# taiyaki-go/motioncheck_ccm_slam

Hardware: AMD Instinct MI355X
Metric: ORB extract+match Mfeatures/s and GBA iter/s (2k KF, 200k pts) @1/2/4/8 GPU (higher is better)
Workload: dtype u8; 1 GPU; configs[1]: 256 synthetic 752x480 frames per GPU, 8-level pyramid, 1000 features, FAST+quadtree+rBRIEF, then 1000x1000 brute-force Hamming on the 255 consecutive pairs; frames_per_gpu=256

## Files before the change

### include/ccm_hot.h

```cpp
#ifndef CCM_HOT_H
#define CCM_HOT_H

#include <stddef.h>
#include <stdint.h>

#ifdef __cplusplus
extern "C" {
#endif

#define CCM_ABI_VERSION 3

enum {
    CCM_OK = 0,
    CCM_E_ARG = -1,
    CCM_E_DEVICE = -2,
    CCM_E_NOMEM = -3,
    CCM_E_CAPACITY = -4,
    CCM_E_NUMERIC = -5,
    CCM_E_COMM = -6,
    CCM_E_STATE = -7
};

typedef struct ccm_ctx ccm_ctx;

int ccm_abi_version(void);
ccm_ctx* ccm_create(int device, int flags);
void ccm_destroy(ccm_ctx*);
const char* ccm_last_error(const ccm_ctx*);
int ccm_sync(ccm_ctx*);
void* ccm_stream(ccm_ctx*);

enum { CCM_PROF_RESIZE = 0, CCM_PROF_FAST_SCORE, CCM_PROF_CELL_NMS, CCM_PROF_OCTREE, CCM_PROF_ORIENT_DESC,
       CCM_PROF_HAMMING_BF,
       CCM_PROF_BA_LINEARIZE, CCM_PROF_BA_DINV_Y, CCM_PROF_BA_SCHUR_BLOCKS, CCM_PROF_BA_BSCHUR, CCM_PROF_BA_BACKSUB,
       CCM_PROF_COUNT };
int ccm_host_register(ccm_ctx*, void* ptr, size_t bytes);
int ccm_host_unregister(ccm_ctx*, void* ptr);

int ccm_profile_enable(ccm_ctx*, int on);
int ccm_profile_read(ccm_ctx*, float ms[CCM_PROF_COUNT], int32_t launches[CCM_PROF_COUNT]);

typedef struct {
    int   nfeatures;
    float scale_factor;
    int   nlevels;
    int   ini_th_fast;
    int   min_th_fast;
} ccm_orb_params;

#define CCM_MAX_LEVELS 16

typedef struct {
    float x, y;
    float size;
    float angle;
    float response;
    int32_t octave;
    int32_t class_id;
} ccm_keypoint;

int ccm_orb_tables(const ccm_orb_params*, float* scale, float* inv_scale, float* sigma2,
                   float* inv_sigma2, int32_t* features_per_level, int32_t* umax);
int ccm_orb_level_sizes(const ccm_orb_params*, int w, int h, int32_t* level_w, int32_t* level_h);

int ccm_orb_extract(ccm_ctx*, const ccm_orb_params*, const uint8_t* img, int w, int h, int stride,
                    size_t image_stride, int n_images, ccm_keypoint* kps, uint8_t* desc,
                    int32_t* counts, int max_per_image);

int ccm_orb_extract_dev(ccm_ctx*, const ccm_orb_params*, const uint8_t* img_dev, int w, int h,
                        int stride, size_t image_stride, int n_images, int max_per_image);
int ccm_orb_fetch(ccm_ctx*, ccm_keypoint* kps, uint8_t* desc, int32_t* counts);
int ccm_orb_result_dev(ccm_ctx*, const uint8_t** desc_dev, const int32_t** counts_dev,
                       int* max_per_image);

int ccm_orb_debug_level(ccm_ctx*, int image, int level, uint8_t* out, int out_stride);
int ccm_orb_debug_candidates(ccm_ctx*, int image, int level, int32_t* xy, int32_t* score, int max);

int ccm_descriptor_distance(const uint8_t* a, const uint8_t* b);

int ccm_hamming_match(ccm_ctx*, const uint8_t* q, int nq, const uint8_t* t, int nt, int n_pairs,
                      const int32_t* nq_n, const int32_t* nt_n,
                      int32_t* best_idx, int32_t* best_dist, int32_t* second_dist);
int ccm_hamming_match_dev(ccm_ctx*, const uint8_t* q_dev, int nq, size_t q_pair_stride,
                          const uint8_t* t_dev, int nt, size_t t_pair_stride, int n_pairs,
                          const int32_t* nq_n_dev, const int32_t* nt_n_dev,
                          int32_t* best_idx_dev, int32_t* best_dist_dev, int32_t* second_dist_dev);

int ccm_ratio_test(int best_dist, int second_dist, float nnratio, int th, int strict);

typedef struct {
    float nnratio;
    int   check_ori;
    int   th;
    int   strict_th;
} ccm_bow_options;
int ccm_match_bow(ccm_ctx*, const ccm_bow_options*,
                  const uint8_t* desc1, const int32_t* node1, const uint8_t* valid1,
                  const float* angle1, int n1,
                  const uint8_t* desc2, const int32_t* node2, const uint8_t* valid2,
                  const float* angle2, int n2, int32_t* match12);

typedef struct {
    int n;
    const float* kp_x; const float* kp_y; const int32_t* kp_octave;
    const uint8_t* desc;
    float min_x, min_y;
    float inv_w, inv_h;
    int grid_cols, grid_rows;
} ccm_frame_grid;
int ccm_window_candidates(ccm_ctx*, const ccm_frame_grid*, int nq, const float* qx, const float* qy, const float* qr,
                          const int32_t* min_level, const int32_t* max_level, const uint8_t* qdesc, int cap,
                          int32_t* cand_idx, int32_t* cand_dist, int32_t* cand_n);
int ccm_search_by_projection(ccm_ctx*, const ccm_frame_grid*, const float* scale_factors, int n_mp, const uint8_t* in_view,
                             const int32_t* level, const float* view_cos, const float* proj_x, const float* proj_y,
                             const uint8_t* mp_desc, const uint8_t* mp_has_obs, uint8_t* occupied, float th, float nnratio,
                             int32_t* match);

int ccm_search_by_projection_frame(ccm_ctx*, const ccm_frame_grid* current, const float* cur_angle, const float* scale_factors,
                                   int n_last, const uint8_t* valid, const float* u, const float* v, const int32_t* last_octave,
                                   const float* last_angle, const uint8_t* mp_desc, const uint8_t* mp_has_obs, uint8_t* occupied,
                                   float th, int check_ori, int orb_dist, int32_t* match);

int ccm_search_for_initialization(ccm_ctx*, int n1, const int32_t* oct1, const uint8_t* desc1, const float* angle1,
                                  const ccm_frame_grid* f2, const float* angle2, float* prev_matched_xy, int window,
                                  float nnratio, int check_ori, int32_t* matches12);

int ccm_fuse_select(ccm_ctx*, const ccm_frame_grid* kf, const float* scale_factors, const float* inv_level_sigma2, int n_mp,
                    const uint8_t* valid, const float* u, const float* v, const int32_t* level, const uint8_t* mp_desc, float th,
                    int chi2_check, int accept_th, int32_t* best_idx, int32_t* best_dist);

int ccm_fuse_select_batch(ccm_ctx*, int n_kf, const ccm_frame_grid* kfs, const float* scale_factors, const float* inv_level_sigma2,
                          const int32_t* mp_first, const uint8_t* valid, const float* u, const float* v, const int32_t* level,
                          const uint8_t* mp_desc, float th, int chi2_check, int accept_th, int32_t* best_idx, int32_t* best_dist);

int ccm_search_by_sim3(ccm_ctx*, const ccm_frame_grid* kf1, const float* scale_factors1, const ccm_frame_grid* kf2, const float* scale_factors2,
                       const uint8_t* valid1, const float* u1, const float* v1, const int32_t* level1, const uint8_t* mp_desc1,
                       const uint8_t* valid2, const float* u2, const float* v2, const int32_t* level2, const uint8_t* mp_desc2,
                       float th, int32_t* match12);

int ccm_search_by_projection_sim3(ccm_ctx*, const ccm_frame_grid* kf, const float* scale_factors, int n_mp, const uint8_t* valid,
                                  const float* u, const float* v, const int32_t* level, const uint8_t* mp_desc, const uint8_t* observed,
                                  uint8_t* matched, float th, int32_t* best_idx);
int ccm_search_by_projection_sim3_batch(ccm_ctx*, int n_kf, const ccm_frame_grid* kfs, const float* scale_factors, const int32_t* mp_first,
                                        const uint8_t* valid, const float* u, const float* v, const int32_t* level, const uint8_t* mp_desc,
                                        const uint8_t* observed, uint8_t* matched, float th, int32_t* best_idx, int32_t* n_matches);

int ccm_search_for_triangulation(ccm_ctx*, const uint8_t* desc1, const int32_t* node1, const uint8_t* has_mp1, const float* x1, const float* y1,
                                 const float* angle1, int n1, const uint8_t* desc2, const int32_t* node2, const uint8_t* has_mp2,
                                 const float* x2, const float* y2, const float* angle2, const int32_t* octave2, int n2, const float* F12,
                                 float ex, float ey, const float* scale_factors2, const float* level_sigma2_2, int check_ori, int32_t* match12);

typedef struct ccm_vocabulary ccm_vocabulary;
int  ccm_voc_create(ccm_ctx*, int k, int L, int n_nodes, const int32_t* parent, const uint8_t* descriptors, const double* weights,
                    ccm_vocabulary** out);
void ccm_voc_destroy(ccm_vocabulary*);
int  ccm_voc_words(const ccm_vocabulary*);

int ccm_voc_transform(ccm_vocabulary*, const uint8_t* features, int n, int levelsup, int32_t* word_id, double* weight, int32_t* node_id);
int ccm_voc_transform_dev(ccm_vocabulary*, const uint8_t* features_dev, int n, int levelsup, int32_t* word_id, double* weight,
                          int32_t* node_id);

int ccm_bow_vector(int n, const int32_t* word_id, const double* weight, const int32_t* node_id, int weighting, int scoring,
                   int32_t* out_id, double* out_val, int32_t* fv_node);
double ccm_bow_score_l1(int n1, const int32_t* id1, const double* v1, int n2, const int32_t* id2, const double* v2);

int ccm_distinctive_descriptors(ccm_vocabulary*, const uint8_t* desc, const int64_t* first, const int32_t* count, int n_points,
                                int32_t* best);

typedef struct {
    int      n_poses;
    double*  poses;
    const uint8_t* fixed;
    const double*  intr;
    int      n_points;
    double*  points;
    int      n_edges;
    const int32_t* edge_pose;
    const int32_t* edge_point;
    const double*  obs;
    const double*  info;
} ccm_ba_problem;

typedef struct {
    int    iterations;
    double huber_delta;
    int    iterations2;
    double outlier_chi2;
    const volatile uint8_t* stop_flag;
    double pcg_tol;
} ccm_ba_options;

typedef struct {
    int    iterations_done;
    int    trials;
    double chi2_initial;
    double chi2_final;
    double lambda_final;
    int    stopped;
    double t_linearize, t_schur, t_solve, t_update;
    uint8_t* edge_outlier;
    int32_t schur_blocks;
    int64_t schur_pairs;
    int32_t pcg_iterations;
    int32_t pcg_fallbacks;
    int32_t pcg_pipelined;
} ccm_ba_result;

int ccm_ba_solve(ccm_ctx*, ccm_ba_problem*, const ccm_ba_options*, ccm_ba_result*);

typedef struct {
    int            n_frames;
    double*        poses;
    const double*  intr;
    const int32_t* first;
    const double*  points;
    const double*  obs;
    const double*  info;
    uint8_t*       outlier;
    int32_t*       n_inliers;
} ccm_pose_problem;
int ccm_pose_optimize(ccm_ctx*, ccm_pose_problem*);

typedef struct ccm_frame ccm_frame;
int ccm_frame_create(ccm_ctx*, const ccm_frame_grid* g, const float* angle, ccm_frame** out);
int ccm_frame_from_extract(ccm_ctx*, int image, int n, const float* kp_x_un, const float* kp_y_un, float min_x, float min_y,
                           float inv_w, float inv_h, int grid_cols, int grid_rows, ccm_frame** out);
void ccm_frame_destroy(ccm_frame*);
int ccm_frame_size(const ccm_frame*);
int ccm_frame_set_map_points(ccm_frame*, const int32_t* mp_id);
int ccm_frame_get_map_points(ccm_frame*, int32_t* mp_id);
int ccm_frame_debug_grid(ccm_frame*, int32_t* cell_first, int32_t* cell_items);
int ccm_frame_search_by_projection(ccm_ctx*, ccm_frame* f, const float* scale_factors, int n_mp, const uint8_t* in_view,
                                   const int32_t* level, const float* view_cos, const float* proj_x, const float* proj_y,
                                   const uint8_t* mp_desc, const uint8_t* mp_has_obs, const int32_t* query_mp_id,
                                   uint8_t* occupied, float th, float nnratio, int32_t* match);
// ... 99 lines not shown
```

### motioncheck_ccm_slam_amd/_lib.py

```python
from __future__ import annotations

import ctypes as C
import os

import numpy as np

_HERE = os.path.dirname(os.path.abspath(__file__))
LIB_PATH = os.environ.get("CCM_HOT_LIB") or os.path.join(_HERE, "libccm_hot.so")

CCM_OK = 0
ERRORS = {-1: "CCM_E_ARG", -2: "CCM_E_DEVICE", -3: "CCM_E_NOMEM", -4: "CCM_E_CAPACITY",
          -5: "CCM_E_NUMERIC", -6: "CCM_E_COMM", -7: "CCM_E_STATE"}
COMM_ID_BYTES = 128

KP_DTYPE = np.dtype([("x", "f4"), ("y", "f4"), ("size", "f4"), ("angle", "f4"), ("response", "f4"),
                     ("octave", "i4"), ("class_id", "i4")])

SYMBOLS = [
    "ccm_abi_version", "ccm_create", "ccm_destroy", "ccm_last_error", "ccm_sync", "ccm_stream",
    "ccm_host_register", "ccm_host_unregister", "ccm_profile_enable", "ccm_profile_read",
    "ccm_orb_tables", "ccm_orb_level_sizes", "ccm_orb_extract", "ccm_orb_extract_dev", "ccm_orb_fetch",
    "ccm_orb_result_dev", "ccm_orb_debug_level", "ccm_orb_debug_candidates",
    "ccm_descriptor_distance", "ccm_hamming_match", "ccm_hamming_match_dev", "ccm_ratio_test", "ccm_match_bow",
    "ccm_window_candidates", "ccm_search_by_projection", "ccm_search_by_projection_frame", "ccm_search_for_initialization", "ccm_fuse_select", "ccm_fuse_select_batch", "ccm_search_by_sim3", "ccm_search_by_projection_sim3", "ccm_search_by_projection_sim3_batch",
    "ccm_search_for_triangulation", "ccm_voc_create", "ccm_voc_destroy", "ccm_voc_words", "ccm_voc_transform", "ccm_voc_transform_dev",
    "ccm_bow_vector", "ccm_bow_score_l1", "ccm_distinctive_descriptors", "ccm_optimize_sim3", "ccm_optimize_essential_graph", "ccm_correct_map_points",
    "ccm_ba_solve", "ccm_ba_landmark_cuts", "ccm_pose_optimize", "ccm_comm_unique_id", "ccm_comm_init", "ccm_comm_attach", "ccm_comm_destroy",
    "ccm_pose_from_mat4f", "ccm_pose_to_mat4f",
    "ccm_frame_create", "ccm_frame_from_extract", "ccm_frame_destroy", "ccm_frame_size", "ccm_frame_set_map_points",
    "ccm_frame_get_map_points", "ccm_frame_debug_grid", "ccm_frame_search_by_projection", "ccm_frame_search_by_projection_frame",
    "ccm_frame_pose_optimize",
    "ccm_sim3_ransac_iterations", "ccm_sim3_solver_create", "ccm_sim3_solver_destroy", "ccm_sim3_solver_count", "ccm_sim3_solver_iterate",
    "ccm_sim3_solver_find", "ccm_sim3_solver_estimate", "ccm_sim3_solver_state", "ccm_sim3_solver_hypotheses",
]


class CcmError(RuntimeError):
    def __init__(self, code, text=""):
        super().__init__("%s (%d): %s" % (ERRORS.get(code, "CCM_E_?"), code, text))
        self.code = code


class OrbParams(C.Structure):
    _fields_ = [("nfeatures", C.c_int), ("scale_factor", C.c_float), ("nlevels", C.c_int),
                ("ini_th_fast", C.c_int), ("min_th_fast", C.c_int)]


class BowOptions(C.Structure):
    _fields_ = [("nnratio", C.c_float), ("check_ori", C.c_int), ("th", C.c_int), ("strict_th", C.c_int)]


class FrameGrid(C.Structure):
    _fields_ = [("n", C.c_int), ("kp_x", C.c_void_p), ("kp_y", C.c_void_p), ("kp_octave", C.c_void_p), ("desc", C.c_void_p),
                ("min_x", C.c_float), ("min_y", C.c_float), ("inv_w", C.c_float), ("inv_h", C.c_float),
                ("grid_cols", C.c_int), ("grid_rows", C.c_int)]


class BaProblem(C.Structure):
    _fields_ = [("n_poses", C.c_int), ("poses", C.c_void_p), ("fixed", C.c_void_p), ("intr", C.c_void_p),
                ("n_points", C.c_int), ("points", C.c_void_p),
                ("n_edges", C.c_int), ("edge_pose", C.c_void_p), ("edge_point", C.c_void_p),
                ("obs", C.c_void_p), ("info", C.c_void_p)]


class PoseProblem(C.Structure):
    _fields_ = [("n_frames", C.c_int), ("poses", C.c_void_p), ("intr", C.c_void_p), ("first", C.c_void_p),
                ("points", C.c_void_p), ("obs", C.c_void_p), ("info", C.c_void_p), ("outlier", C.c_void_p),
                ("n_inliers", C.c_void_p)]


class Sim3Problem(C.Structure):
    _fields_ = [("n_problems", C.c_int), ("sim3", C.c_void_p), ("fix_scale", C.c_void_p), ("K1", C.c_void_p), ("K2", C.c_void_p),
                ("first", C.c_void_p), ("P1", C.c_void_p), ("P2", C.c_void_p), ("obs1", C.c_void_p), ("obs2", C.c_void_p),
                ("info1", C.c_void_p), ("info2", C.c_void_p), ("th2", C.c_void_p), ("inlier", C.c_void_p), ("n_inliers", C.c_void_p)]


class Sim3RansacProblem(C.Structure):
    _fields_ = [("n_solvers", C.c_int32), ("first", C.c_void_p), ("n1", C.c_void_p), ("fix_scale", C.c_void_p), ("K1", C.c_void_p),
                ("K2", C.c_void_p), ("X1", C.c_void_p), ("X2", C.c_void_p), ("max_err1", C.c_void_p), ("max_err2", C.c_void_p),
                ("indices1", C.c_void_p), ("probability", C.c_double), ("min_inliers", C.c_int32), ("max_iterations", C.c_int32),
                ("draws", C.c_void_p), ("best_inliers", C.c_void_p)]


class EssentialGraph(C.Structure):
    _fields_ = [("n_vertices", C.c_int), ("sim3", C.c_void_p), ("fixed", C.c_void_p), ("fix_scale", C.c_int), ("n_edges", C.c_int),
                ("edge_i", C.c_void_p), ("edge_j", C.c_void_p), ("measurement", C.c_void_p), ("iterations", C.c_int),
                ("iterations_done", C.c_int), ("chi2_initial", C.c_double), ("chi2_final", C.c_double),
                ("factor_blocks", C.c_int), ("factor_rounds", C.c_int), ("solver_bytes", C.c_int64)]


class BaOptions(C.Structure):
    _fields_ = [("iterations", C.c_int), ("huber_delta", C.c_double), ("iterations2", C.c_int),
                ("outlier_chi2", C.c_double), ("stop_flag", C.c_void_p), ("pcg_tol", C.c_double)]


class BaResult(C.Structure):
    _fields_ = [("iterations_done", C.c_int), ("trials", C.c_int), ("chi2_initial", C.c_double),
                ("chi2_final", C.c_double), ("lambda_final", C.c_double), ("stopped", C.c_int),
                ("t_linearize", C.c_double), ("t_schur", C.c_double), ("t_solve", C.c_double),
                ("t_update", C.c_double), ("edge_outlier", C.c_void_p),
                ("schur_blocks", C.c_int32), ("schur_pairs", C.c_int64), ("pcg_iterations", C.c_int32),
                ("pcg_fallbacks", C.c_int32), ("pcg_pipelined", C.c_int32)]


ABI_VERSION = 3
_lib = None


def load():
    global _lib
    if _lib is not None:
        return _lib
    if not os.path.exists(LIB_PATH):
        raise ImportError("%s not found: build it with `make -C motioncheck_ccm_slam_amd/csrc` "
                          "(or __graft_entry__.build()); there is no CPU fallback" % LIB_PATH)
    lib = C.CDLL(LIB_PATH)
    if lib.ccm_abi_version() != ABI_VERSION:
        raise ImportError("%s has ABI version %d, this package mirrors version %d of include/ccm_hot.h: rebuild it"
                          % (LIB_PATH, lib.ccm_abi_version(), ABI_VERSION))
    lib.ccm_create.restype = C.c_void_p
    lib.ccm_create.argtypes = [C.c_int, C.c_int]
    lib.ccm_destroy.argtypes = [C.c_void_p]
    lib.ccm_destroy.restype = None
    lib.ccm_last_error.restype = C.c_char_p
    lib.ccm_last_error.argtypes = [C.c_void_p]
    lib.ccm_sync.argtypes = [C.c_void_p]
    lib.ccm_stream.restype = C.c_void_p
    lib.ccm_stream.argtypes = [C.c_void_p]
    vp = C.c_void_p
    lib.ccm_host_register.argtypes = [vp, vp, C.c_size_t]
    lib.ccm_host_unregister.argtypes = [vp, vp]
    lib.ccm_profile_enable.argtypes = [vp, C.c_int]
    lib.ccm_profile_read.argtypes = [vp, vp, vp]
    lib.ccm_orb_tables.argtypes = [C.POINTER(OrbParams)] + [vp] * 6
    lib.ccm_orb_level_sizes.argtypes = [C.POINTER(OrbParams), C.c_int, C.c_int, vp, vp]
    lib.ccm_orb_extract.argtypes = [vp, C.POINTER(OrbParams), vp, C.c_int, C.c_int, C.c_int, C.c_size_t, C.c_int,
                                    vp, vp, vp, C.c_int]
    lib.ccm_orb_extract_dev.argtypes = [vp, C.POINTER(OrbParams), vp, C.c_int, C.c_int, C.c_int, C.c_size_t,
                                        C.c_int, C.c_int]
    lib.ccm_orb_fetch.argtypes = [vp, vp, vp, vp]
    lib.ccm_orb_result_dev.argtypes = [vp, C.POINTER(vp), C.POINTER(vp), C.POINTER(C.c_int)]
    lib.ccm_orb_debug_level.argtypes = [vp, C.c_int, C.c_int, vp, C.c_int]
    lib.ccm_orb_debug_candidates.argtypes = [vp, C.c_int, C.c_int, vp, vp, C.c_int]
    lib.ccm_descriptor_distance.argtypes = [vp, vp]
    lib.ccm_hamming_match.argtypes = [vp, vp, C.c_int, vp, C.c_int, C.c_int, vp, vp, vp, vp, vp]
    lib.ccm_hamming_match_dev.argtypes = [vp, vp, C.c_int, C.c_size_t, vp, C.c_int, C.c_size_t, C.c_int,
                                          vp, vp, vp, vp, vp]
    lib.ccm_ratio_test.argtypes = [C.c_int, C.c_int, C.c_float, C.c_int, C.c_int]
    lib.ccm_match_bow.argtypes = [vp, C.POINTER(BowOptions), vp, vp, vp, vp, C.c_int, vp, vp, vp, vp, C.c_int, vp]
    lib.ccm_window_candidates.argtypes = [vp, C.POINTER(FrameGrid), C.c_int, vp, vp, vp, vp, vp, vp, C.c_int, vp, vp, vp]
    lib.ccm_search_by_projection.argtypes = [vp, C.POINTER(FrameGrid), vp, C.c_int, vp, vp, vp, vp, vp, vp, vp, vp, C.c_float, C.c_float, vp]
    lib.ccm_search_by_projection_frame.argtypes = [vp, C.POINTER(FrameGrid), vp, vp, C.c_int, vp, vp, vp, vp, vp, vp, vp, vp, C.c_float, C.c_int, C.c_int, vp]
    lib.ccm_search_for_initialization.argtypes = [vp, C.c_int, vp, vp, vp, C.POINTER(FrameGrid), vp, vp, C.c_int, C.c_float, C.c_int, vp]
    lib.ccm_fuse_select.argtypes = [vp, C.POINTER(FrameGrid), vp, vp, C.c_int, vp, vp, vp, vp, vp, C.c_float, C.c_int, C.c_int, vp, vp]
    lib.ccm_fuse_select_batch.argtypes = [vp, C.c_int, vp, vp, vp, vp, vp, vp, vp, vp, vp, C.c_float, C.c_int, C.c_int, vp, vp]
    lib.ccm_search_by_sim3.argtypes = [vp, C.POINTER(FrameGrid), vp, C.POINTER(FrameGrid), vp] + [vp] * 10 + [C.c_float, vp]
    lib.ccm_search_by_projection_sim3.argtypes = [vp, C.POINTER(FrameGrid), vp, C.c_int] + [vp] * 7 + [C.c_float, vp]
    lib.ccm_search_by_projection_sim3_batch.argtypes = [vp, C.c_int, vp, vp, vp] + [vp] * 7 + [C.c_float, vp, vp]
    lib.ccm_search_for_triangulation.argtypes = [vp] * 7 + [C.c_int] + [vp] * 7 + [C.c_int, vp, C.c_float, C.c_float, vp, vp, C.c_int, vp]
    lib.ccm_voc_create.argtypes = [vp, C.c_int, C.c_int, C.c_int, vp, vp, vp, C.POINTER(vp)]
    lib.ccm_voc_destroy.argtypes = [vp]; lib.ccm_voc_destroy.restype = None
    lib.ccm_voc_words.argtypes = [vp]
    lib.ccm_voc_transform.argtypes = [vp, vp, C.c_int, C.c_int, vp, vp, vp]
    lib.ccm_voc_transform_dev.argtypes = [vp, vp, C.c_int, C.c_int, vp, vp, vp]
    lib.ccm_bow_vector.argtypes = [C.c_int, vp, vp, vp, C.c_int, C.c_int, vp, vp, vp]
    lib.ccm_bow_score_l1.argtypes = [C.c_int, vp, vp, C.c_int, vp, vp]; lib.ccm_bow_score_l1.restype = C.c_double
    lib.ccm_distinctive_descriptors.argtypes = [vp, vp, vp, vp, C.c_int, vp]
    lib.ccm_ba_solve.argtypes = [vp, C.POINTER(BaProblem), C.POINTER(BaOptions), C.POINTER(BaResult)]
    lib.ccm_ba_landmark_cuts.argtypes = [vp, C.c_int, C.c_int, C.c_int, vp]
    lib.ccm_comm_attach.argtypes = [vp, vp, C.c_int, C.c_int]
    lib.ccm_pose_optimize.argtypes = [vp, C.POINTER(PoseProblem)]
    lib.ccm_optimize_sim3.argtypes = [vp, C.POINTER(Sim3Problem)]
    lib.ccm_optimize_essential_graph.argtypes = [vp, C.POINTER(EssentialGraph)]
    lib.ccm_correct_map_points.argtypes = [vp, C.c_int, vp, vp, C.c_int, vp, vp]
    lib.ccm_comm_unique_id.argtypes = [vp]
    lib.ccm_comm_init.argtypes = [vp, vp, C.c_int, C.c_int]
    lib.ccm_comm_destroy.argtypes = [vp]
    lib.ccm_pose_from_mat4f.argtypes = [vp, vp]
    lib.ccm_pose_to_mat4f.argtypes = [vp, vp]
    lib.ccm_frame_create.argtypes = [vp, C.POINTER(FrameGrid), vp, C.POINTER(vp)]
    lib.ccm_frame_from_extract.argtypes = [vp, C.c_int, C.c_int, vp, vp, C.c_float, C.c_float, C.c_float, C.c_float, C.c_int, C.c_int,
                                           C.POINTER(vp)]
    lib.ccm_frame_destroy.argtypes = [vp]; lib.ccm_frame_destroy.restype = None
    lib.ccm_frame_size.argtypes = [vp]
    lib.ccm_frame_set_map_points.argtypes = [vp, vp]
    lib.ccm_frame_get_map_points.argtypes = [vp, vp]
    lib.ccm_frame_debug_grid.argtypes = [vp, vp, vp]
    lib.ccm_frame_search_by_projection.argtypes = [vp, vp, vp, C.c_int] + [vp] * 9 + [C.c_float, C.c_float, vp]
    lib.ccm_frame_search_by_projection_frame.argtypes = [vp, vp, vp, vp, C.c_int] + [vp] * 9 + [C.c_float, C.c_int, C.c_int, vp]
    lib.ccm_frame_pose_optimize.argtypes = [vp, vp, C.c_int, vp, vp, C.c_int, vp, vp, vp, vp]
    lib.ccm_sim3_ransac_iterations.argtypes = [C.c_int, C.c_double, C.c_int, C.c_int]
    lib.ccm_sim3_solver_create.argtypes = [vp, C.POINTER(Sim3RansacProblem), C.POINTER(vp)]
    lib.ccm_sim3_solver_destroy.argtypes = [vp]; lib.ccm_sim3_solver_destroy.restype = None
    lib.ccm_sim3_solver_count.argtypes = [vp]
    lib.ccm_sim3_solver_iterate.argtypes = [vp, C.c_int, C.c_int, vp, vp, vp, vp, vp]
    lib.ccm_sim3_solver_find.argtypes = [vp, C.c_int, vp, vp, vp, vp]
    lib.ccm_sim3_solver_estimate.argtypes = [vp, C.c_int, vp, vp, vp]
    lib.ccm_sim3_solver_state.argtypes = [vp, C.c_int, vp, vp, vp, vp]
    lib.ccm_sim3_solver_hypotheses.argtypes = [vp, C.c_int, vp, vp, vp, vp]
    _lib = lib
    return lib


def ptr(a):
    if a is None:
        return None
    if isinstance(a, int):
        return C.c_void_p(a)
    return a.ctypes.data_as(C.c_void_p)


class Context:

    def __init__(self, device: int = 0):
        self.lib = load()
        self.handle = self.lib.ccm_create(int(device), 0)
        if not self.handle:
            raise CcmError(-2, "ccm_create(%d) failed: no such HIP device" % device)
        self.device = device

    def check(self, rc: int) -> int:
        if rc < 0:
            raise CcmError(rc, self.lib.ccm_last_error(self.handle).decode(errors="replace"))
        return rc

    PROF_LABELS = ("k_pyr_resize", "k_fast_score", "k_cell_nms", "k_octree", "k_orient_desc", "k_hamming_bf",
                   "ba_linearize", "ba_dinv_y", "k_sp_schur_blocks", "k_sp_bschur", "k_ba_backsub")

    def host_register(self, arr):
        self.check(self.lib.ccm_host_register(self.handle, ptr(arr), C.c_size_t(arr.nbytes)))

    def host_unregister(self, arr):
        self.check(self.lib.ccm_host_unregister(self.handle, ptr(arr)))

    def profile(self, on: bool):
        self.check(self.lib.ccm_profile_enable(self.handle, int(on)))

    def profile_read(self):
        ms = np.zeros(len(self.PROF_LABELS), "f4"); n = np.zeros(len(self.PROF_LABELS), "i4")
        self.check(self.lib.ccm_profile_read(self.handle, ptr(ms), ptr(n)))
        return {k: (float(ms[i]), int(n[i])) for i, k in enumerate(self.PROF_LABELS)}

    def sync(self):
        self.check(self.lib.ccm_sync(self.handle))

    @property
    def stream(self) -> int:
        return self.lib.ccm_stream(self.handle)

    def close(self):
        if getattr(self, "handle", None):
            self.lib.ccm_destroy(self.handle)
            self.handle = None

    def __del__(self):
        try:
            self.close()
        except Exception:
            pass


_default_ctx = {}


def default_context(device: int = 0) -> Context:
    if device not in _default_ctx:
        _default_ctx[device] = Context(device)
    return _default_ctx[device]
```

### motioncheck_ccm_slam_amd/csrc/match_host.cpp

```cpp
#include "ccm_internal.h"
#include "window_types.h"
#include <algorithm>
#include <climits>
#include <cmath>
#include <numeric>

void match_launch_bf(hipStream_t, const uint8_t* q, long long q_pair_bytes, const uint8_t* t, long long t_pair_bytes,
                     int nq, int nt, int n_pairs, const int* nq_n, const int* nt_n, int n_split, int variant,
                     unsigned* part_best, int* part_second, int* bi, int* bd, int* sd);
void match_launch_ranges(hipStream_t, const uint8_t* d1, const uint8_t* d2, const int* order2, const int* start,
                         const int* len, const long long* off, int n1, unsigned short* dist);
struct BowDev {
    int n_groups, n1;
    const int* ga; const int* gae; const int* gb; const int* gbe;
    const int* ord1; const int* ord2;
    const uint8_t* d1; const uint8_t* d2;
    const uint8_t* valid1; const uint8_t* valid2;
    const float* angle1; const float* angle2;
    uint8_t* taken; int* match12; int* bin_of; int* hist;
    float nnratio; int th, strict_th, check_ori;
};
void match_launch_bow(hipStream_t, const BowDev&);

struct WindowBufs { DevBuf kx, ky, oct, desc, cfirst, citems, qx, qy, qr, minl, maxl, qdesc, ci, cd, cn, sel_i, sel_d, is2, act, qlvl, qflag, flag, out, status, qang, fang, ev,
                           grids, qkf, gkf; };
struct MatchState {
    WindowBufs win;
    DevBuf q, t, nqn, ntn, bi, bd, sd;
    DevBuf part_best, part_second;
    DevBuf d1, d2, order2, start, len, off, dist;
    DevBuf order1, grp[4], bv1, bv2, ba1, ba2, taken, m12, binof, hist;
};
void match_state_free(MatchState* s) { delete s; }

static MatchState* match_state(ccm_ctx* c)
{
    if (!c->match) c->match = new MatchState();
    return c->match;
}
static WindowBufs& window_bufs(ccm_ctx* c) { return match_state(c)->win; }

extern "C" {

int ccm_descriptor_distance(const uint8_t* a, const uint8_t* b)
{
    int d = 0;
    for (int i = 0; i < 8; i++) {
        uint32_t x, y;
        std::memcpy(&x, a + 4 * i, 4);
        std::memcpy(&y, b + 4 * i, 4);
        d += __builtin_popcount(x ^ y);
    }
    return d;
}

int ccm_ratio_test(int best_dist, int second_dist, float nnratio, int th, int strict)
{
    const bool pass = strict ? (best_dist < th) : (best_dist <= th);
    return pass && (static_cast<float>(best_dist) < nnratio * static_cast<float>(second_dist)) ? 1 : 0;
}

int ccm_hamming_match_dev(ccm_ctx* c, const uint8_t* q_dev, int nq, size_t q_pair_stride, const uint8_t* t_dev, int nt,
                          size_t t_pair_stride, int n_pairs, const int32_t* nq_n_dev, const int32_t* nt_n_dev,
                          int32_t* best_idx_dev, int32_t* best_dist_dev, int32_t* second_dist_dev)
{
    RoctxRange roctx_("ccm_hamming_match_dev");
    return ccm_guard(c, "ccm_hamming_match_dev", [&]() -> int {
        if (!c) return CCM_E_ARG;
        if (n_pairs == 0 || nq == 0) return CCM_OK;
        if (n_pairs < 0 || nq < 0 || nt < 0 || nt > 65535 || !q_dev || (!t_dev && nt > 0) || !best_idx_dev || !best_dist_dev || !second_dist_dev)
            return ccm_fail(c, CCM_E_ARG, "bad matcher arguments (nt must be <= 65535)");
        if (((uintptr_t)q_dev | (uintptr_t)t_dev) & 15) return ccm_fail(c, CCM_E_ARG, "descriptor arrays must be 16-byte aligned");
        CCM_HIP(c, hipSetDevice(c->device));
        MatchState& M = *match_state(c);
        static const int env_split = getenv("CCM_BF_SPLIT") ? atoi(getenv("CCM_BF_SPLIT")) : 0;
        static const int variant = getenv("CCM_BF_VARIANT") ? atoi(getenv("CCM_BF_VARIANT")) : 3;
        int n_split = env_split > 0 ? env_split : 1;
        if (env_split <= 0) while (n_split < 8 && (long long)n_pairs * n_split < 1024 && nt / (n_split * 2) >= 128) n_split *= 2;
        if (n_split > 1) {
            CCM_RESERVE(c, M.part_best, (size_t)n_pairs * n_split * nq * 4);
            CCM_RESERVE(c, M.part_second, (size_t)n_pairs * n_split * nq * 4);
        }
        ProfScope ps(c, CCM_PROF_HAMMING_BF);
        match_launch_bf(c->stream, q_dev, (long long)q_pair_stride * 32, t_dev, (long long)t_pair_stride * 32, nq, nt, n_pairs,
                        nq_n_dev, nt_n_dev, n_split, variant, M.part_best.as<unsigned>(), M.part_second.as<int>(),
                        best_idx_dev, best_dist_dev, second_dist_dev);
        CCM_HIP(c, hipGetLastError());
        return CCM_OK;
    });
}

int ccm_hamming_match(ccm_ctx* c, const uint8_t* q, int nq, const uint8_t* t, int nt, int n_pairs, const int32_t* nq_n,
                      const int32_t* nt_n, int32_t* best_idx, int32_t* best_dist, int32_t* second_dist)
{
    RoctxRange roctx_("ccm_hamming_match");
    return ccm_guard(c, "ccm_hamming_match", [&]() -> int {
        if (!c) return CCM_E_ARG;
        if (n_pairs == 0 || nq == 0) return CCM_OK;
        if (n_pairs < 0 || nq < 0 || nt < 0 || !q || (!t && nt > 0) || !best_idx || !best_dist || !second_dist)
            return ccm_fail(c, CCM_E_ARG, "bad matcher arguments");
        CCM_HIP(c, hipSetDevice(c->device));
        MatchState& M = *match_state(c);
        const size_t qb = (size_t)n_pairs * nq * 32, tb = (size_t)n_pairs * nt * 32, ob = (size_t)n_pairs * nq * 4;
        CCM_RESERVE(c, M.q, qb); CCM_RESERVE(c, M.t, std::max<size_t>(tb, 32));
        CCM_RESERVE(c, M.bi, ob); CCM_RESERVE(c, M.bd, ob); CCM_RESERVE(c, M.sd, ob);
        CCM_RESERVE(c, M.nqn, (size_t)n_pairs * 4); CCM_RESERVE(c, M.ntn, (size_t)n_pairs * 4);
        CCM_HIP(c, hipMemcpyAsync(M.q.p, q, qb, hipMemcpyHostToDevice, c->stream));
        if (tb) CCM_HIP(c, hipMemcpyAsync(M.t.p, t, tb, hipMemcpyHostToDevice, c->stream));
        if (nq_n) CCM_HIP(c, hipMemcpyAsync(M.nqn.p, nq_n, (size_t)n_pairs * 4, hipMemcpyHostToDevice, c->stream));
        if (nt_n) CCM_HIP(c, hipMemcpyAsync(M.ntn.p, nt_n, (size_t)n_pairs * 4, hipMemcpyHostToDevice, c->stream));
        int rc = ccm_hamming_match_dev(c, M.q.as<uint8_t>(), nq, nq, M.t.as<uint8_t>(), nt, nt, n_pairs,
                                       nq_n ? M.nqn.as<int32_t>() : nullptr, nt_n ? M.ntn.as<int32_t>() : nullptr,
                                       M.bi.as<int32_t>(), M.bd.as<int32_t>(), M.sd.as<int32_t>());
        if (rc) return rc;
        CCM_HIP(c, hipMemcpyAsync(best_idx, M.bi.p, ob, hipMemcpyDeviceToHost, c->stream));
        CCM_HIP(c, hipMemcpyAsync(best_dist, M.bd.p, ob, hipMemcpyDeviceToHost, c->stream));
        CCM_HIP(c, hipMemcpyAsync(second_dist, M.sd.p, ob, hipMemcpyDeviceToHost, c->stream));
        CCM_HIP(c, hipStreamSynchronize(c->stream));
        return CCM_OK;
    });
}

static void three_maxima(const std::vector<int>* histo, int L, int& ind1, int& ind2, int& ind3)
{
    int max1 = 0, max2 = 0, max3 = 0;
    ind1 = ind2 = ind3 = -1;
    for (int i = 0; i < L; i++) {
        const int s = (int)histo[i].size();
        if (s > max1) { max3 = max2; max2 = max1; max1 = s; ind3 = ind2; ind2 = ind1; ind1 = i; }
        else if (s > max2) { max3 = max2; max2 = s; ind3 = ind2; ind2 = i; }
        else if (s > max3) { max3 = s; ind3 = i; }
    }
    if (max2 < 0.1f * (float)max1) { ind2 = -1; ind3 = -1; }
    else if (max3 < 0.1f * (float)max1) { ind3 = -1; }
}

struct RotHisto {
    static const int HISTO = 30;
    std::vector<int> rot[HISTO];
    void add(float r, int idx)
    {
        if (r < 0.0) r += 360.0f;
        int bin = (int)std::round(r * (1.0f / HISTO));
        if (bin == HISTO) bin = 0;
        rot[bin].push_back(idx);
    }
    std::vector<int> outliers() const
    {
        int i1, i2, i3;
        three_maxima(rot, HISTO, i1, i2, i3);
        std::vector<int> out;
        for (int b = 0; b < HISTO; b++)
            if (b != i1 && b != i2 && b != i3) out.insert(out.end(), rot[b].begin(), rot[b].end());
        return out;
    }
};

struct BowRanges {
    std::vector<int> ord1, ord2, start, len;
    std::vector<long long> off;
    std::vector<unsigned short> dist;
};
static int bow_ranges(ccm_ctx* c, const uint8_t* desc1, const int32_t* node1, const uint8_t* valid1, int n1,
                      const uint8_t* desc2, const int32_t* node2, int n2, BowRanges& R)
{
    MatchState& M = *match_state(c);
    std::vector<int>&ord1 = R.ord1, &ord2 = R.ord2, &start = R.start, &len = R.len;
    std::vector<long long>& off = R.off;
    std::vector<unsigned short>& dist = R.dist;
    ord1.assign(n1, 0); ord2.assign(n2, 0);
    std::iota(ord1.begin(), ord1.end(), 0); std::iota(ord2.begin(), ord2.end(), 0);
    auto by_node = [](const int32_t* node) { return [node](int a, int b) { return node[a] != node[b] ? node[a] < node[b] : a < b; }; };
    std::stable_sort(ord1.begin(), ord1.end(), by_node(node1));
    std::stable_sort(ord2.begin(), ord2.end(), by_node(node2));
    start.assign(n1, 0); len.assign(n1, 0); off.assign(n1 + 1, 0);
    {
        size_t b = 0;
        for (size_t a = 0; a < ord1.size();) {
            const int nd = node1[ord1[a]];
            size_t ae = a; while (ae < ord1.size() && node1[ord1[ae]] == nd) ae++;
            while (b < ord2.size() && node2[ord2[b]] < nd) b++;
            size_t be = b; while (be < ord2.size() && node2[ord2[be]] == nd) be++;
            if (nd >= 0) for (size_t i = a; i < ae; i++) if (valid1[ord1[i]]) { start[ord1[i]] = (int)b; len[ord1[i]] = (int)(be - b); }
            a = ae; b = be;
        }
    }
    for (int i = 0; i < n1; i++) off[i + 1] = off[i] + len[i];
    const long long total = off[n1];
    dist.assign((size_t)std::max<long long>(total, 1), 0);
    if (total > 0) {
        CCM_RESERVE(c, M.d1, (size_t)n1 * 32); CCM_RESERVE(c, M.d2, (size_t)n2 * 32);
        CCM_RESERVE(c, M.order2, (size_t)n2 * 4); CCM_RESERVE(c, M.start, (size_t)n1 * 4); CCM_RESERVE(c, M.len, (size_t)n1 * 4);
        CCM_RESERVE(c, M.off, (size_t)(n1 + 1) * 8); CCM_RESERVE(c, M.dist, (size_t)total * 2);
        CCM_HIP(c, hipMemcpyAsync(M.d1.p, desc1, (size_t)n1 * 32, hipMemcpyHostToDevice, c->stream));
        CCM_HIP(c, hipMemcpyAsync(M.d2.p, desc2, (size_t)n2 * 32, hipMemcpyHostToDevice, c->stream));
        CCM_HIP(c, hipMemcpyAsync(M.order2.p, ord2.data(), (size_t)n2 * 4, hipMemcpyHostToDevice, c->stream));
        CCM_HIP(c, hipMemcpyAsync(M.start.p, start.data(), (size_t)n1 * 4, hipMemcpyHostToDevice, c->stream));
        CCM_HIP(c, hipMemcpyAsync(M.len.p, len.data(), (size_t)n1 * 4, hipMemcpyHostToDevice, c->stream));
        CCM_HIP(c, hipMemcpyAsync(M.off.p, off.data(), (size_t)(n1 + 1) * 8, hipMemcpyHostToDevice, c->stream));
        match_launch_ranges(c->stream, M.d1.as<uint8_t>(), M.d2.as<uint8_t>(), M.order2.as<int>(), M.start.as<int>(),
                            M.len.as<int>(), M.off.as<long long>(), n1, M.dist.as<unsigned short>());
        CCM_HIP(c, hipGetLastError());
        CCM_HIP(c, hipMemcpyAsync(dist.data(), M.dist.p, (size_t)total * 2, hipMemcpyDeviceToHost, c->stream));
        CCM_HIP(c, hipStreamSynchronize(c->stream));
    }
    return CCM_OK;
}

int ccm_match_bow(ccm_ctx* c, const ccm_bow_options* o, const uint8_t* desc1, const int32_t* node1, const uint8_t* valid1,
                  const float* angle1, int n1, const uint8_t* desc2, const int32_t* node2, const uint8_t* valid2,
                  const float* angle2, int n2, int32_t* match12)
{
    RoctxRange roctx_("ccm_match_bow");
    return ccm_guard(c, "ccm_match_bow", [&]() -> int {
        if (!c || !o) return CCM_E_ARG;
        if (n1 < 0 || n2 < 0 || (n1 > 0 && (!desc1 || !node1 || !valid1 || !match12)) || (n2 > 0 && (!desc2 || !node2)) ||
            (o->check_ori && n1 > 0 && n2 > 0 && (!angle1 || !angle2)))
            return ccm_fail(c, CCM_E_ARG, "bad SearchByBoW arguments");
        for (int i = 0; i < n1; i++) match12[i] = -1;
        if (n1 == 0 || n2 == 0) return 0;
        CCM_HIP(c, hipSetDevice(c->device));
        MatchState& M = *match_state(c);
        std::vector<int> ord1(n1), ord2(n2);
        std::iota(ord1.begin(), ord1.end(), 0); std::iota(ord2.begin(), ord2.end(), 0);
        auto by_node = [](const int32_t* node) { return [node](int a, int b) { return node[a] != node[b] ? node[a] < node[b] : a < b; }; };
        std::stable_sort(ord1.begin(), ord1.end(), by_node(node1));
        std::stable_sort(ord2.begin(), ord2.end(), by_node(node2));
        std::vector<int> grp[4];
        {
            size_t pa = 0, pb = 0;
            while (pa < ord1.size() && pb < ord2.size()) {
                const int na = node1[ord1[pa]], nb2 = node2[ord2[pb]];
                if (na < 0) { pa++; continue; }
                if (nb2 < 0) { pb++; continue; }
                if (na < nb2) { while (pa < ord1.size() && node1[ord1[pa]] == na) pa++; continue; }
                if (nb2 < na) { while (pb < ord2.size() && node2[ord2[pb]] == nb2) pb++; continue; }
                size_t ae = pa, be = pb;
                while (ae < ord1.size() && node1[ord1[ae]] == na) ae++;
                while (be < ord2.size() && node2[ord2[be]] == na) be++;
                grp[0].push_back((int)pa); grp[1].push_back((int)ae); grp[2].push_back((int)pb); grp[3].push_back((int)be);
                pa = ae; pb = be;
            }
        }
        const int ng = (int)grp[0].size();
        hipStream_t st = c->stream;
        int rc;
        if ((rc = ccm_upload(c, M.d1, desc1, (size_t)n1 * 32, st)) || (rc = ccm_upload(c, M.d2, desc2, (size_t)n2 * 32, st))) return rc;
        if ((rc = ccm_upload(c, M.order1, ord1.data(), (size_t)n1 * 4, st)) || (rc = ccm_upload(c, M.order2, ord2.data(), (size_t)n2 * 4, st))) return rc;
        for (int k = 0; k < 4; k++) if ((rc = ccm_upload(c, M.grp[k], grp[k].data(), (size_t)ng * 4, st))) return rc;
        if ((rc = ccm_upload(c, M.bv1, valid1, (size_t)n1, st))) return rc;
        if (valid2 && (rc = ccm_upload(c, M.bv2, valid2, (size_t)n2, st))) return rc;
        if (o->check_ori && ((rc = ccm_upload(c, M.ba1, angle1, (size_t)n1 * 4, st)) || (rc = ccm_upload(c, M.ba2, angle2, (size_t)n2 * 4, st)))) return rc;
        CCM_RESERVE(c, M.taken, (size_t)n2); CCM_RESERVE(c, M.m12, (size_t)n1 * 4); CCM_RESERVE(c, M.binof, (size_t)n1 * 4); CCM_RESERVE(c, M.hist, 32 * 4);
        CCM_HIP(c, hipMemsetAsync(M.taken.p, 0, (size_t)n2, st));
        CCM_HIP(c, hipMemsetAsync(M.m12.p, 0xFF, (size_t)n1 * 4, st));
        CCM_HIP(c, hipMemsetAsync(M.hist.p, 0, 32 * 4, st));
        BowDev B{ ng, n1, M.grp[0].as<int>(), M.grp[1].as<int>(), M.grp[2].as<int>(), M.grp[3].as<int>(), M.order1.as<int>(), M.order2.as<int>(),
                  M.d1.as<uint8_t>(), M.d2.as<uint8_t>(), M.bv1.as<uint8_t>(), valid2 ? M.bv2.as<uint8_t>() : nullptr,
                  M.ba1.as<float>(), M.ba2.as<float>(), M.taken.as<uint8_t>(), M.m12.as<int>(), M.binof.as<int>(), M.hist.as<int>(),
                  o->nnratio, o->th, o->strict_th, o->check_ori };
        match_launch_bow(st, B);
        CCM_HIP(c, hipGetLastError());
        int nmatches = 0;
        CCM_HIP(c, hipMemcpyAsync(match12, M.m12.p, (size_t)n1 * 4, hipMemcpyDeviceToHost, st));
        CCM_HIP(c, hipMemcpyAsync(&nmatches, M.hist.as<int>() + 30, 4, hipMemcpyDeviceToHost, st));
        CCM_HIP(c, hipStreamSynchronize(st));
        return nmatches;
    });
}

// ... 659 lines not shown
```

### motioncheck_ccm_slam_amd/csrc/match_kernels.hip

```cpp
#include <hip/hip_runtime.h>
#include <cstdint>

#define BF_TILE 1024

__device__ __forceinline__ int ham256(const uint4& a0, const uint4& a1, const uint4& b0, const uint4& b1)
{
    int d = __popc(a0.x ^ b0.x);
    d += __popc(a0.y ^ b0.y); d += __popc(a0.z ^ b0.z); d += __popc(a0.w ^ b0.w);
    d += __popc(a1.x ^ b1.x); d += __popc(a1.y ^ b1.y); d += __popc(a1.z ^ b1.z); d += __popc(a1.w ^ b1.w);
    return d;
}

template <int THREADS, int QPL>
__global__ __launch_bounds__(THREADS) void k_hamming_bf(
    const uint8_t* __restrict__ q, long long q_pair_bytes, const uint8_t* __restrict__ t, long long t_pair_bytes,
    int nq, int nt, const int* __restrict__ nq_n, const int* __restrict__ nt_n, int n_split,
    unsigned* __restrict__ part_best, int* __restrict__ part_second,
    int* __restrict__ best_idx, int* __restrict__ best_dist, int* __restrict__ second_dist)
{
    __shared__ uint4 tile[BF_TILE * 2];
    const int pair = blockIdx.x / n_split, split = blockIdx.x - pair * n_split, tid = threadIdx.x;
    const int nqp = nq_n ? min(max(nq_n[pair], 0), nq) : nq;
    const int ntp = nt_n ? min(max(nt_n[pair], 0), nt) : nt;
    const int chunk = ((ntp + n_split - 1) / n_split + 63) & ~63;
    const int t_lo = min(split * chunk, ntp), t_hi = min(t_lo + chunk, ntp);
    const uint4* qp = reinterpret_cast<const uint4*>(q + (long long)pair * q_pair_bytes);
    const uint4* tp = reinterpret_cast<const uint4*>(t + (long long)pair * t_pair_bytes);
    const int q_done = ((nqp + QPL * THREADS - 1) / (QPL * THREADS)) * (QPL * THREADS);
    if (n_split == 1 || split == 0)
        for (int qi = q_done + tid; qi < nq; qi += THREADS) {
            if (n_split > 1) {
                for (int sp = 0; sp < n_split; sp++) {
                    const long long o = ((long long)pair * n_split + sp) * nq + qi;
                    part_best[o] = (256u << 16) | 0xFFFFu; part_second[o] = 256;
                }
            } else {
                const long long o = (long long)pair * nq + qi;
                best_idx[o] = -1; best_dist[o] = 256; second_dist[o] = 256;
            }
        }
    for (int qbase = 0; qbase < nqp; qbase += QPL * THREADS) {
        uint4 a0[QPL], a1[QPL];
        unsigned best[QPL]; int sec[QPL];
#pragma unroll
        for (int k = 0; k < QPL; k++) {
            const int qi = qbase + k * THREADS + tid;
            a0[k] = make_uint4(0, 0, 0, 0); a1[k] = a0[k];
            if (qi < nqp) { a0[k] = qp[2 * qi]; a1[k] = qp[2 * qi + 1]; }
            best[k] = (256u << 16) | 0xFFFFu; sec[k] = 256;
        }
        for (int tbase = t_lo; tbase < t_hi; tbase += BF_TILE) {
            const int cnt = min(BF_TILE, t_hi - tbase);
            __syncthreads();
            for (int i = tid; i < 2 * cnt; i += THREADS) tile[i] = tp[2 * tbase + i];
            __syncthreads();
#pragma unroll 2
            for (int j = 0; j < cnt; j++) {
                const uint4 b0 = tile[2 * j], b1 = tile[2 * j + 1];
                const unsigned idx = (unsigned)(tbase + j);
#pragma unroll
                for (int k = 0; k < QPL; k++) {
                    const int d = ham256(a0[k], a1[k], b0, b1);
                    sec[k] = min(sec[k], max(d, (int)(best[k] >> 16)));
                    best[k] = min(best[k], ((unsigned)d << 16) | idx);
                }
            }
        }
#pragma unroll
        for (int k = 0; k < QPL; k++) {
            const int qi = qbase + k * THREADS + tid;
            if (qi >= nq) continue;
            if (n_split > 1) {
                const long long o = ((long long)pair * n_split + split) * nq + qi;
                part_best[o] = best[k]; part_second[o] = sec[k];
            } else {
                const bool live = qi < nqp;
                const long long o = (long long)pair * nq + qi;
                best_idx[o] = (live && (best[k] >> 16) < 256u) ? (int)(best[k] & 0xFFFFu) : -1;
                best_dist[o] = live ? (int)(best[k] >> 16) : 256;
                second_dist[o] = live ? sec[k] : 256;
            }
        }
    }
}

typedef int hm_v4i __attribute__((ext_vector_type(4)));
typedef int hm_v16i __attribute__((ext_vector_type(16)));
#ifndef HM_CB
#define HM_CB 2
#endif
#ifndef HM_WAVES
#define HM_WAVES 4
#endif
#ifndef HM_TT
#define HM_TT 1
#endif
#ifndef HM_WG_PER_CU
#define HM_WG_PER_CU 4
#endif
#define HM_QW (32 * HM_CB)
#define HM_TPB (64 * HM_WAVES)
#define HM_SENT 0x3FFFFFFF
#define HM_MAX_NT 2048

#define HM_BIAS 4352
#define HM_IDX_BITS 11
__device__ __forceinline__ int hm_med3(int a, int b, int c)
{
    return __float_as_int(__builtin_amdgcn_fmed3f(__int_as_float(a), __int_as_float(b), __int_as_float(c)));
}

__device__ __forceinline__ hm_v4i hm_expand16(unsigned hw, int shift)
{
    hm_v4i v;
    const unsigned hs = hw << shift, nm = 15u << shift, bm = 0x01010101u << shift;
    v.x = (int)(__umul24(hs & nm, 0x204081u) & bm); v.y = (int)(__umul24((hs >> 4) & nm, 0x204081u) & bm);
    v.z = (int)(__umul24((hs >> 8) & nm, 0x204081u) & bm); v.w = (int)(__umul24((hs >> 12) & nm, 0x204081u) & bm);
    return v;
}

__global__ __launch_bounds__(HM_TPB, HM_WG_PER_CU * HM_TPB / 256) void k_hamming_mfma(
    const uint8_t* __restrict__ q, long long q_pair_bytes, const uint8_t* __restrict__ t, long long t_pair_bytes,
    int nq, int nt, const int* __restrict__ nq_n, const int* __restrict__ nt_n, int q_blocks,
    int* __restrict__ best_idx, int* __restrict__ best_dist, int* __restrict__ second_dist)
{
    __shared__ hm_v4i frag[2][HM_TT * 8][64];
    __shared__ __attribute__((aligned(16))) int wall[HM_MAX_NT];
    const int pair = blockIdx.x / q_blocks, qblk = blockIdx.x - pair * q_blocks;
    const int tid = threadIdx.x, lane = tid & 63, wv = tid >> 6, h = lane >> 5, r = lane & 31;
    const int nqp = nq_n ? min(max(nq_n[pair], 0), nq) : nq;
    const int ntp = nt_n ? min(max(nt_n[pair], 0), nt) : nt;
    const unsigned* qp = reinterpret_cast<const unsigned*>(q + (long long)pair * q_pair_bytes);
    const unsigned* tp = reinterpret_cast<const unsigned*>(t + (long long)pair * t_pair_bytes);
    const int q0 = qblk * (HM_QW * HM_WAVES) + wv * HM_QW;
    if (qblk * (HM_QW * HM_WAVES) >= nqp) {
        for (int i = tid; i < HM_QW * HM_WAVES; i += HM_TPB) {
            const int qi = qblk * (HM_QW * HM_WAVES) + i;
            if (qi < nq) { const long long o = (long long)pair * nq + qi; best_idx[o] = -1; best_dist[o] = 256; second_dist[o] = 256; }
        }
        return;
    }

    hm_v4i bq[HM_CB][8];
    int pa[HM_CB];
#pragma unroll
    for (int cb = 0; cb < HM_CB; cb++) {
        const int qi = q0 + 32 * cb + r;
        unsigned d[8];
        int pc = 0;
#pragma unroll
        for (int s = 0; s < 8; s++) { d[s] = qi < nqp ? qp[8 * (long long)qi + s] : 0u; pc += __popc(d[s]); }
        pa[cb] = pc;
#pragma unroll
        for (int s = 0; s < 8; s++) bq[cb][s] = hm_expand16((d[s] >> (16 * h)) & 0xFFFFu, 7);
    }
    int m1[HM_CB], m2[HM_CB];
#pragma unroll
    for (int cb = 0; cb < HM_CB; cb++) { m1[cb] = HM_SENT; m2[cb] = HM_SENT; }

    constexpr int HM_FPT = (512 * HM_TT + HM_TPB - 1) / HM_TPB;
    struct Raw { unsigned v[HM_FPT]; };
    auto fetch = [&](int group) {
        Raw x;
#pragma unroll
        for (int j = 0; j < HM_FPT; j++) {
            const int fi = tid + j * HM_TPB, sub = fi >> 9, fw = fi & 511;
            const int tr = (group * HM_TT + sub) * 32 + (fw & 31);
            x.v[j] = (fi < 512 * HM_TT && tr < ntp) ? tp[8 * (long long)tr + ((fw >> 5) & 7)] : 0u;
        }
        return x;
    };
    auto stage = [&](const Raw& x, int buf) {
#pragma unroll
        for (int j = 0; j < HM_FPT; j++) {
            const int fi = tid + j * HM_TPB, sub = fi >> 9, fw = fi & 511;
            if (fi < 512 * HM_TT) frag[buf][8 * sub + ((fw >> 5) & 7)][32 * (fw >> 8) + (fw & 31)] = hm_expand16((x.v[j] >> (16 * (fw >> 8))) & 0xFFFFu, 5);
        }
    };
    for (int tr = tid; tr < ((ntp + 31) & ~31); tr += HM_TPB) {
        int w = HM_SENT;
        if (tr < ntp) {
            const uint4* d = reinterpret_cast<const uint4*>(tp + 8 * (long long)tr);
            const uint4 d0 = d[0], d1 = d[1];
            const int pb = __popc(d0.x) + __popc(d0.y) + __popc(d0.z) + __popc(d0.w) + __popc(d1.x) + __popc(d1.y) + __popc(d1.z) + __popc(d1.w);
            w = ((pb + HM_BIAS) << HM_IDX_BITS) | tr;
        }
        wall[tr] = w;
    }
    const int ntiles = (ntp + 31) >> 5;
    const bool wave_live = q0 < nqp;
    auto mma = [&](int tile, int buf, int sub, hm_v16i (&acc)[HM_CB]) {
        hm_v16i wc;
#pragma unroll
        for (int g = 0; g < 4; g++) {
            const hm_v4i w4 = *reinterpret_cast<const hm_v4i*>(&wall[32 * tile + 8 * g + 4 * h]);
            wc[4 * g] = w4.x; wc[4 * g + 1] = w4.y; wc[4 * g + 2] = w4.z; wc[4 * g + 3] = w4.w;
        }
#pragma unroll
        for (int s = 0; s < 8; s++) {
            const hm_v4i a = frag[buf][8 * sub + s][lane];
#pragma unroll
            for (int cb = 0; cb < HM_CB; cb++) acc[cb] = __builtin_amdgcn_mfma_i32_32x32x32_i8(a, bq[cb][s], s == 0 ? wc : acc[cb], 0, 0, 0);
        }
    };
    auto fold = [&](const hm_v16i (&acc)[HM_CB]) {
#pragma unroll
        for (int i = 0; i < 16; i++)
#pragma unroll
            for (int cb = 0; cb < HM_CB; cb++) {
                const int kx = acc[cb][i];
                m2[cb] = hm_med3(m1[cb], m2[cb], kx); m1[cb] = min(m1[cb], kx);
            }
    };
    const int ngroups = (ntiles + HM_TT - 1) / HM_TT;
    Raw nxt = fetch(0);
    if (ngroups > 0) stage(nxt, 0);
    nxt = fetch(1);
    __syncthreads();
    for (int grp = 0; grp < ngroups; grp++) {
        const int buf = grp & 1;
        if (grp + 1 < ngroups) stage(nxt, buf ^ 1);
        if (grp + 2 < ngroups) nxt = fetch(grp + 2);
        if (wave_live) {
#pragma unroll
            for (int sub = 0; sub < HM_TT; sub++) {
                const int tile = grp * HM_TT + sub;
                if (tile < ntiles) {
                    hm_v16i acc[HM_CB];
                    mma(tile, buf, sub, acc);
                    fold(acc);
                }
            }
        }
        __syncthreads();
    }
#pragma unroll
    for (int cb = 0; cb < HM_CB; cb++) {
        const int o1 = __shfl_xor(m1[cb], 32, 64), o2 = __shfl_xor(m2[cb], 32, 64);
        const int b1 = min(m1[cb], o1);
        const int b2 = min(max(m1[cb], o1), min(m2[cb], o2));
        const int qi = q0 + 32 * cb + r;
        if (h == 0 && qi < nq) {
            const long long o = (long long)pair * nq + qi;
            const bool live = qi < nqp;
            const bool has1 = live && b1 < HM_SENT, has2 = live && b2 < HM_SENT;
            const int bd = has1 ? (b1 >> HM_IDX_BITS) - HM_BIAS + pa[cb] : 256;
            best_idx[o] = bd < 256 ? (b1 & ((1 << HM_IDX_BITS) - 1)) : -1;
            best_dist[o] = bd;
            second_dist[o] = has2 ? (b2 >> HM_IDX_BITS) - HM_BIAS + pa[cb] : 256;
        }
    }
}

__global__ __launch_bounds__(256) void k_hamming_merge(const unsigned* __restrict__ part_best, const int* __restrict__ part_second,
                                                       int n_pairs, int nq, int n_split, const int* __restrict__ nq_n,
                                                       int* __restrict__ best_idx, int* __restrict__ best_dist, int* __restrict__ second_dist)
{
    const long long i = blockIdx.x * 256LL + threadIdx.x;
    if (i >= (long long)n_pairs * nq) return;
    const int pair = (int)(i / nq), qi = (int)(i - (long long)pair * nq);
    const int nqp = nq_n ? min(max(nq_n[pair], 0), nq) : nq;
    unsigned best = (256u << 16) | 0xFFFFu; int sec = 256;
    for (int s = 0; s < n_split; s++) {
        const long long o = ((long long)pair * n_split + s) * nq + qi;
        const unsigned b = part_best[o]; const int sc = part_second[o];
        sec = min(min(sec, sc), max((int)(best >> 16), (int)(b >> 16)));
        best = min(best, b);
    }
    const bool live = qi < nqp;
    best_idx[i] = (live && (best >> 16) < 256u) ? (int)(best & 0xFFFFu) : -1;
    best_dist[i] = live ? (int)(best >> 16) : 256;
    second_dist[i] = live ? sec : 256;
}

__global__ __launch_bounds__(256) void k_hamming_ranges(
    const uint8_t* __restrict__ d1, const uint8_t* __restrict__ d2, const int* __restrict__ order2,
    const int* __restrict__ start, const int* __restrict__ len, const long long* __restrict__ off, int n1,
    unsigned short* __restrict__ dist)
{
    const int i = blockIdx.x * 4 + (threadIdx.x >> 6), lane = threadIdx.x & 63;
    if (i >= n1) return;
    const int L = len[i];
    if (L <= 0) return;
    const uint4* a = reinterpret_cast<const uint4*>(d1) + 2 * (long long)i;
    const uint4 a0 = a[0], a1 = a[1];
    const int s = start[i];
    unsigned short* o = dist + off[i];
    for (int k = lane; k < L; k += 64) {
        const uint4* b = reinterpret_cast<const uint4*>(d2) + 2 * (long long)order2[s + k];
        o[k] = (unsigned short)ham256(a0, a1, b[0], b[1]);
    }
}

struct BowDev {
    int n_groups, n1;
    const int* ga; const int* gae; const int* gb; const int* gbe;
    const int* ord1; const int* ord2;
    const uint8_t* d1b; const uint8_t* d2b;
    const uint8_t* valid1; const uint8_t* valid2;
    const float* angle1; const float* angle2;
    uint8_t* taken; int* match12; int* bin_of; int* hist;
    float nnratio; int th, strict_th, check_ori;
};
__global__ __launch_bounds__(256) void k_bow_greedy(BowDev B)
{
    const int grp = blockIdx.x * 4 + (threadIdx.x >> 6), lane = threadIdx.x & 63;
    if (grp >= B.n_groups) return;
    const int a0 = B.ga[grp], a1 = B.gae[grp], b0 = B.gb[grp], b1 = B.gbe[grp];
    for (int a = a0; a < a1; a++) {
        const int i1 = B.ord1[a];
        if (!B.valid1[i1]) continue;
        const uint4* D1 = reinterpret_cast<const uint4*>(B.d1b); const uint4* D2 = reinterpret_cast<const uint4*>(B.d2b);
        const uint4 q0 = D1[2 * (long long)i1], q1 = D1[2 * (long long)i1 + 1];
        int bd1 = 256, bd2 = 256, bi = -1;
        for (int base = b0; base < b1; base += 64) {
            const int j = base + lane;
            int d = 1 << 20, i2 = -1;
            if (j < b1) {
                i2 = B.ord2[j];
                if (!B.taken[i2] && (!B.valid2 || B.valid2[i2])) d = ham256(q0, q1, D2[2 * (long long)i2], D2[2 * (long long)i2 + 1]);
            }
            unsigned key = ((unsigned)d << 6) | (unsigned)lane;
#pragma unroll
            for (int s = 32; s >= 1; s >>= 1) key = min(key, (unsigned)__shfl_xor((int)key, s, 64));
            const int cb = (int)(key >> 6), cl = (int)(key & 63u);
            int o = lane == cl ? (1 << 20) : d;
#pragma unroll
            for (int s = 32; s >= 1; s >>= 1) o = min(o, __shfl_xor(o, s, 64));
            const int ci2 = __shfl(i2, cl, 64);
            if (cb < bd1) { bd2 = min(bd1, o); bd1 = cb; bi = ci2; }
            else bd2 = min(bd2, cb);
        }
        const bool pass = B.strict_th ? (bd1 < B.th) : (bd1 <= B.th);
        if (bi >= 0 && pass && (float)bd1 < B.nnratio * (float)bd2) {
            if (lane == 0) {
                B.match12[i1] = bi;
                B.taken[bi] = 1;
                if (B.check_ori) {
                    float r = B.angle1[i1] - B.angle2[bi];
                    if (r < 0.0) r += 360.0f;
                    int bin = (int)roundf(r * (1.0f / 30));
                    if (bin == 30) bin = 0;
                    B.bin_of[i1] = bin;
                    atomicAdd(&B.hist[bin], 1);
                }
            }
            __threadfence_block();
        }
    }
}
__global__ __launch_bounds__(256) void k_bow_filter(BowDev B)
{
    __shared__ int keep[3];
    __shared__ int cnt;
    if (threadIdx.x == 0) {
        int max1 = 0, max2 = 0, max3 = 0, ind1 = -1, ind2 = -1, ind3 = -1;
        if (B.check_ori) {
            for (int i = 0; i < 30; i++) {
                const int s = B.hist[i];
                if (s > max1) { max3 = max2; max2 = max1; max1 = s; ind3 = ind2; ind2 = ind1; ind1 = i; }
                else if (s > max2) { max3 = max2; max2 = s; ind3 = ind2; ind2 = i; }
                else if (s > max3) { max3 = s; ind3 = i; }
            }
            if (max2 < 0.1f * (float)max1) { ind2 = -1; ind3 = -1; }
            else if (max3 < 0.1f * (float)max1) ind3 = -1;
        }
        keep[0] = ind1; keep[1] = ind2; keep[2] = ind3; cnt = 0;
    }
    __syncthreads();
    int mine = 0;
    for (int i = threadIdx.x; i < B.n1; i += 256) {
        if (B.match12[i] < 0) continue;
        if (B.check_ori) {
            const int b = B.bin_of[i];
            if (b != keep[0] && b != keep[1] && b != keep[2]) { B.match12[i] = -1; continue; }
        }
        mine++;
    }
    atomicAdd(&cnt, mine);
    __syncthreads();
    if (threadIdx.x == 0) B.hist[30] = cnt;
}
void match_launch_bow(hipStream_t s, const BowDev& B)
{
    if (B.n_groups > 0) hipLaunchKernelGGL(k_bow_greedy, dim3((B.n_groups + 3) / 4), dim3(256), 0, s, B);
    hipLaunchKernelGGL(k_bow_filter, dim3(1), dim3(256), 0, s, B);
}

struct WinGrid {
    int n, cols, rows;
    float min_x, min_y, inv_w, inv_h;
    const float* kx; const float* ky; const int* oct; const uint8_t* desc;
    const int* cell_first; const int* cell_items;
};
template <bool BATCH>
__global__ __launch_bounds__(256) void k_window_candidates(WinGrid G1, const WinGrid* __restrict__ grids, const int* __restrict__ q_kf,
                                                           int nq, const float* __restrict__ qx, const float* __restrict__ qy,
                                                           const float* __restrict__ qr, const int* __restrict__ min_level,
                                                           const int* __restrict__ max_level, const uint8_t* __restrict__ qdesc, int cap,
                                                           int* __restrict__ cand_idx, int* __restrict__ cand_dist, int* __restrict__ cand_n)
{
    const int q = blockIdx.x * 4 + (threadIdx.x >> 6), lane = threadIdx.x & 63;
    if (q >= nq) return;
    const WinGrid G = BATCH ? grids[q_kf[q]] : G1;
// ... 195 lines not shown
                }
            }
            sync(wg);
            const int th = MODE == 0 ? 100 : (MODE == 1 ? 50 : A.orb_dist);
            const int bestDist = k1 == 0xFFFFFFFFu ? 256 : (int)(k1 >> 16);
            int idx1 = -1, idx2 = -1;
            bool safe = false;
            if (unres) {
                if (bestDist > th) safe = true;
                else {
                    const int p1 = (int)(k1 & 0xFFFFu), p2 = (int)(k2 & 0xFFFFu);
                    if (p1 >= WG_REG_CAND) idx1 = ci[p1];
                    if (MODE == 0 && k2 != 0xFFFFFFFFu && p2 >= WG_REG_CAND) idx2 = ci[p2];
#pragma unroll
                    for (int k = 0; k < WG_REG_CAND; k++) {
                        if (k == p1) idx1 = (int)(cand[k] & 0xFFFFu);
                        if (MODE == 0 && k2 != 0xFFFFFFFFu && k == p2) idx2 = (int)(cand[k] & 0xFFFFu);
                    }
                    safe = claim[idx1] == me;
                    if (MODE == 0 && idx2 >= 0) safe = safe && claim[idx2] == me;
                }
            }
            sync(wg);
            if (unres) {
#pragma unroll
                for (int k = 0; k < WG_REG_CAND; k++) if (k < c) claim[cand[k] & 0xFFFFu] = 0x7FFFFFFF;
                for (int k = WG_REG_CAND; k < c; k++) claim[ci[k]] = 0x7FFFFFFF;
            }
            if (unres && safe) {
                unres = false;
                if (bestDist <= th) {
                    if (MODE == 0) {
                        const int bestLevel = octl[idx1], bestLevel2 = idx2 >= 0 ? (int)octl[idx2] : -1;
                        const int bestDist2 = idx2 >= 0 ? (int)(k2 >> 16) : 256;
                        if (!(bestLevel == bestLevel2 && bestDist > A.nnratio * bestDist2)) { A.out[idx1] = m; flag[idx1] = (uint8_t)qf; mine++; }
                    } else if (MODE == 1) {
                        A.out[m] = idx1;
                        if (!qf) { flag[idx1] = 1; mine++; }
                    } else {
                        A.out[idx1] = m;
                        flag[idx1] = (uint8_t)qf;
                        int bin = 255;
                        if (A.check_ori) {
                            float rot = A.q_angle[m] - A.f_angle[idx1];
                            if (rot < 0.0) rot += 360.0f;
                            bin = (int)roundf(rot * (1.0f / 30));
                            if (bin == 30) bin = 0;
                        }
                        A.ev[m] = (idx1 << 8) | bin;
                        mine++;
                    }
                }
            }
        };
        int left = 1, rounds = 0;
        for (int r = 0; r < WG_BATCH_ROUNDS && left; r++) {
            round(tid, true);
            left = __syncthreads_count(unres ? 1 : 0);
            rounds++;
        }
        if (left) {
            for (int turn = 0; turn < 16; turn++) {
                if (wv == turn) {
                    while (__ballot(unres) != 0ull) {
                        rounds++;
                        round(lane, false);
                        __builtin_amdgcn_s_waitcnt(0xc07f);
                        __builtin_amdgcn_wave_barrier();
                    }
                }
                __syncthreads();
            }
        }
        most = max(most, rounds);
    }
    if (mine) atomicAdd(&s_count, mine);
    atomicMax(&s_rounds, most);
    __syncthreads();
    if (MODE == 2 && A.check_ori) {
        __shared__ int hist[30], keep3[3], s_removed;
        if (tid < 30) hist[tid] = 0;
        if (tid == 0) s_removed = 0;
        __syncthreads();
        for (int m = tid; m < A.nq; m += 1024) { const int e = (A.active[m] && A.cn[m] > 0) ? A.ev[m] : -1; if (e >= 0) atomicAdd(&hist[e & 255], 1); }
        __syncthreads();
        if (tid == 0) {
            int max1 = 0, max2 = 0, max3 = 0, i1 = -1, i2 = -1, i3 = -1;
            for (int i = 0; i < 30; i++) {
                const int sz = hist[i];
                if (sz > max1) { max3 = max2; max2 = max1; max1 = sz; i3 = i2; i2 = i1; i1 = i; }
                else if (sz > max2) { max3 = max2; max2 = sz; i3 = i2; i2 = i; }
                else if (sz > max3) { max3 = sz; i3 = i; }
            }
            if (max2 < 0.1f * (float)max1) { i2 = -1; i3 = -1; }
            else if (max3 < 0.1f * (float)max1) { i3 = -1; }
            keep3[0] = i1; keep3[1] = i2; keep3[2] = i3;
        }
        __syncthreads();
        int removed = 0;
        for (int m = tid; m < A.nq; m += 1024) {
            const int e = (A.active[m] && A.cn[m] > 0) ? A.ev[m] : -1;
            if (e < 0) continue;
            const int b = e & 255;
            if (b != keep3[0] && b != keep3[1] && b != keep3[2]) { A.out[e >> 8] = -1; removed++; }
        }
        if (removed) atomicAdd(&s_removed, removed);
        __syncthreads();
        if (tid == 0) s_count -= s_removed;
        __syncthreads();
    }
    for (int i = tid; i < A.n; i += 1024) A.flag[i] = flag[i];
    if (tid == 0) { A.status[0] = s_count; A.status[1] = s_maxcn; A.status[2] = s_rounds; }
}
size_t match_window_greedy_lds(int n, int nq) { (void)nq; return (size_t)4 * n + 2 * (size_t)((n + 3) & ~3) + 16; }
int match_launch_window_greedy_batch(hipStream_t s, const GreedyArgs& A, int n_kf, int max_n)
{
    const size_t lds = match_window_greedy_lds(max_n, 0);
    if (hipFuncSetAttribute((const void*)k_window_greedy<1>, hipFuncAttributeMaxDynamicSharedMemorySize, (int)lds) != hipSuccess) return -1;
    hipLaunchKernelGGL(k_window_greedy<1>, dim3(n_kf), dim3(1024), lds, s, A);
    return 0;
}
int match_launch_window_greedy(hipStream_t s, int mode, const GreedyArgs& A)
{
    const size_t lds = match_window_greedy_lds(A.n, A.nq);
    if (mode == 0) {
        if (hipFuncSetAttribute((const void*)k_window_greedy<0>, hipFuncAttributeMaxDynamicSharedMemorySize, (int)lds) != hipSuccess) return -1;
        hipLaunchKernelGGL(k_window_greedy<0>, dim3(1), dim3(1024), lds, s, A);
    } else if (mode == 1) {
        if (hipFuncSetAttribute((const void*)k_window_greedy<1>, hipFuncAttributeMaxDynamicSharedMemorySize, (int)lds) != hipSuccess) return -1;
        hipLaunchKernelGGL(k_window_greedy<1>, dim3(1), dim3(1024), lds, s, A);
    } else {
        if (hipFuncSetAttribute((const void*)k_window_greedy<2>, hipFuncAttributeMaxDynamicSharedMemorySize, (int)lds) != hipSuccess) return -1;
        hipLaunchKernelGGL(k_window_greedy<2>, dim3(1), dim3(1024), lds, s, A);
    }
    return 0;
}

void match_launch_window(hipStream_t s, const WinGrid& G, int nq, const float* qx, const float* qy, const float* qr, const int* minl,
                         const int* maxl, const uint8_t* qdesc, int cap, int* ci, int* cd, int* cn)
{
    hipLaunchKernelGGL(k_window_candidates<false>, dim3((nq + 3) / 4), dim3(256), 0, s, G, (const WinGrid*)nullptr, (const int*)nullptr, nq, qx, qy, qr, minl, maxl, qdesc, cap,
                       ci, cd, cn);
}
void match_launch_window_batch(hipStream_t s, const WinGrid* grids, const int* q_kf, int nq, const float* qx, const float* qy, const float* qr, const int* minl,
                               const int* maxl, const uint8_t* qdesc, int cap, int* ci, int* cd, int* cn)
{
    if (nq > 0) hipLaunchKernelGGL(k_window_candidates<true>, dim3((nq + 3) / 4), dim3(256), 0, s, WinGrid{}, grids, q_kf, nq, qx, qy, qr, minl, maxl, qdesc, cap, ci, cd, cn);
}

void match_launch_bf(hipStream_t s, const uint8_t* q, long long q_pair_bytes, const uint8_t* t, long long t_pair_bytes,
                     int nq, int nt, int n_pairs, const int* nq_n, const int* nt_n, int n_split, int variant,
                     unsigned* part_best, int* part_second, int* bi, int* bd, int* sd)
{
    if (variant == 3 && nt <= HM_MAX_NT) {
        const int q_blocks = (nq + HM_QW * HM_WAVES - 1) / (HM_QW * HM_WAVES);
        hipLaunchKernelGGL(k_hamming_mfma, dim3(n_pairs * q_blocks), dim3(HM_TPB), 0, s, q, q_pair_bytes, t, t_pair_bytes, nq, nt, nq_n, nt_n,
                           q_blocks, bi, bd, sd);
        return;
    }
    const dim3 grid(n_pairs * n_split);
    if (variant == 1)
        hipLaunchKernelGGL((k_hamming_bf<256, 4>), grid, dim3(256), 0, s, q, q_pair_bytes, t, t_pair_bytes, nq, nt, nq_n, nt_n, n_split, part_best, part_second, bi, bd, sd);
    else if (variant == 2)
        hipLaunchKernelGGL((k_hamming_bf<1024, 1>), grid, dim3(1024), 0, s, q, q_pair_bytes, t, t_pair_bytes, nq, nt, nq_n, nt_n, n_split, part_best, part_second, bi, bd, sd);
    else
        hipLaunchKernelGGL((k_hamming_bf<512, 2>), grid, dim3(512), 0, s, q, q_pair_bytes, t, t_pair_bytes, nq, nt, nq_n, nt_n, n_split, part_best, part_second, bi, bd, sd);
    if (n_split > 1)
        hipLaunchKernelGGL(k_hamming_merge, dim3((unsigned)(((long long)n_pairs * nq + 255) / 256)), dim3(256), 0, s,
                           part_best, part_second, n_pairs, nq, n_split, nq_n, bi, bd, sd);
}
void match_launch_ranges(hipStream_t s, const uint8_t* d1, const uint8_t* d2, const int* order2, const int* start,
                         const int* len, const long long* off, int n1, unsigned short* dist)
{
    hipLaunchKernelGGL(k_hamming_ranges, dim3((n1 + 3) / 4), dim3(256), 0, s, d1, d2, order2, start, len, off, n1, dist);
}
```

### motioncheck_ccm_slam_amd/csrc/orb_host.cpp

```cpp
#include "ccm_internal.h"
#include "orb_types.h"
#include <cmath>
#include <cfloat>
#include <algorithm>

extern "C" hipError_t orb_upload_pattern();
size_t orb_octree_lds_bytes(int list_cap);
void orb_launch_resize(hipStream_t, const OrbGeom&, int level, int dw, int dh, int nframes);
void orb_launch_score(hipStream_t, const OrbGeom&, int ntiles, int nframes);
void orb_launch_nms(hipStream_t, const OrbGeom&, const OrbCell*, int ncells, int nframes, unsigned* slots, int* cell_count);
void orb_launch_fast_cells(hipStream_t, const OrbGeom&, const OrbCell*, const OrbBand*, int nbands, int nframes, size_t lds_bytes,
                           int surv_cap, unsigned* slots, int* cell_count);
size_t orb_fast_cells_lds(int pitch, int bh, int surv_cap);
void orb_launch_octree(hipStream_t, const OrbGeom&, const OrbCell*, int nlevels, int nframes, int list_cap,
                       const unsigned* slots, const int* cell_count, unsigned* keysA, unsigned* keysB,
                       unsigned* out, int* out_count, int* status);
void orb_launch_orient_desc(hipStream_t, const OrbGeom&, int out_per_frame, int nframes, const unsigned* sel,
                            const int* sel_count, ccm_keypoint* kps, uint8_t* desc, int* counts, int max_per_image,
                            int* status);

namespace {

inline int cv_round(float v) { return (int)lrintf(v); }
inline int cv_round(double v) { return (int)lrint(v); }

struct OrbTables {
    float scale[ORB_MAX_LEVELS], inv_scale[ORB_MAX_LEVELS], sigma2[ORB_MAX_LEVELS], inv_sigma2[ORB_MAX_LEVELS];
    int nfeat[ORB_MAX_LEVELS];
    int umax[16];
};

int make_tables(const ccm_orb_params* p, OrbTables* t)
{
    if (!p || p->nlevels < 1 || p->nlevels > ORB_MAX_LEVELS || p->nfeatures < 0 || !(p->scale_factor > 1.0f)) return CCM_E_ARG;
    const int n = p->nlevels;
    t->scale[0] = 1.0f; t->sigma2[0] = 1.0f;
    for (int i = 1; i < n; i++) {
        t->scale[i] = t->scale[i - 1] * p->scale_factor;
        t->sigma2[i] = t->scale[i] * t->scale[i];
    }
    for (int i = 0; i < n; i++) {
        t->inv_scale[i] = 1.0f / t->scale[i];
        t->inv_sigma2[i] = 1.0f / t->sigma2[i];
    }
    const float factor = 1.0f / p->scale_factor;
    float desired = p->nfeatures * (1 - factor) / (1 - (float)std::pow((double)factor, (double)n));
    int sum = 0;
    for (int l = 0; l < n - 1; l++) {
        t->nfeat[l] = cv_round(desired);
        sum += t->nfeat[l];
        desired *= factor;
    }
    t->nfeat[n - 1] = std::max(p->nfeatures - sum, 0);
    const int vmax = (int)std::floor(ORB_HALF_PATCH * std::sqrt(2.f) / 2 + 1);
    const int vmin = (int)std::ceil(ORB_HALF_PATCH * std::sqrt(2.f) / 2);
    const double hp2 = ORB_HALF_PATCH * ORB_HALF_PATCH;
    for (int v = 0; v < 16; v++) t->umax[v] = 0;
    for (int v = 0; v <= vmax; ++v) t->umax[v] = cv_round(std::sqrt(hp2 - v * v));
    for (int v = ORB_HALF_PATCH, v0 = 0; v >= vmin; --v) {
        while (t->umax[v0] == t->umax[v0 + 1]) ++v0;
        t->umax[v] = v0;
        ++v0;
    }
    return CCM_OK;
}

void linear_tables(int ssize, int dsize, std::vector<int>& ofs, std::vector<short>& ab)
{
    ofs.resize(dsize); ab.resize(2 * (size_t)dsize);
    const double inv_scale = (double)dsize / ssize;
    const double scale = 1. / inv_scale;
    for (int d = 0; d < dsize; d++) {
        float fx = (float)((d + 0.5) * scale - 0.5);
        int sx = (int)std::floor(fx);
        fx -= sx;
        if (sx < 0) { sx = 0; fx = 0.f; }
        if (sx >= ssize - 1) { sx = ssize - 1; fx = 0.f; }
        ofs[d] = sx;
        ab[2 * d] = (short)cv_round((1.f - fx) * 2048.f);
        ab[2 * d + 1] = (short)cv_round(fx * 2048.f);
    }
}

}

struct OrbState {
    ccm_orb_params par{}; int w = 0, h = 0, nframes = 0, max_per_image = 0;
    bool valid = false, pattern_up = false;
    OrbTables tab{};
    OrbGeom geom{};
    std::vector<OrbCell> cells;
    std::vector<OrbBand> bands; size_t band_lds = 0; bool fused = true; int surv_cap = 1024; hipStream_t copy_stream = nullptr; hipEvent_t copy_done = nullptr;
    hipStream_t down_stream = nullptr; hipEvent_t chunk_done = nullptr;
    DevBuf geom_dev, cells_dev, tables_dev, bands_dev;
    DevBuf pyr, smap, slots, cell_count, keysA, keysB, sel, sel_count, status;
    DevBuf img0;
    DevBuf kps, desc, counts;
    size_t pyr_off[ORB_MAX_LEVELS]{}, smap_off[ORB_MAX_LEVELS]{};
    const uint8_t* last_img = nullptr; int last_stride = 0; size_t last_image_stride = 0;
    bool have_result = false;
};

void orb_state_free(OrbState* s)
{
    if (!s) return;
    if (s->copy_done) (void)hipEventDestroy(s->copy_done);
    if (s->chunk_done) (void)hipEventDestroy(s->chunk_done);
    delete s;
}

static inline size_t align_up(size_t v, size_t a) { return (v + a - 1) / a * a; }

static int orb_prepare(ccm_ctx* c, const ccm_orb_params* p, int w, int h, int nframes, int max_per_image)
{
    if (!c->orb) c->orb = new OrbState();
    OrbState& S = *c->orb;
    const bool same = S.valid && std::memcmp(&S.par, p, sizeof *p) == 0 && S.w == w && S.h == h &&
                      S.nframes == nframes && S.max_per_image == max_per_image;
    if (same) return CCM_OK;
    S.valid = false; S.have_result = false;
    int rc = make_tables(p, &S.tab);
    if (rc) return ccm_fail(c, rc, "bad ORB parameters");
    if (p->ini_th_fast < 0 || p->ini_th_fast > 255 || p->min_th_fast < 0 || p->min_th_fast > 255)
        return ccm_fail(c, CCM_E_ARG, "FAST thresholds must be in [0,255]");
    OrbGeom& G = S.geom;
    std::memset(&G, 0, sizeof G);
    G.nlevels = p->nlevels; G.ini_th = p->ini_th_fast; G.min_th = p->min_th_fast;
    for (int i = 0; i < 16; i++) G.umax[i] = S.tab.umax[i];
    S.cells.clear();
    std::vector<int> tab_i; std::vector<short> tab_s;
    struct TabOff { size_t xofs, yofs, xab, yab; } toff[ORB_MAX_LEVELS]{};
    size_t pyr_bytes = 0, smap_bytes = 0;
    int slot_acc = 0, key_acc = 0, out_acc = 0, tile_acc = 0, max_quota = 0;
    for (int l = 0; l < p->nlevels; l++) {
        OrbLevel& L = G.lv[l];
        L.w = cv_round((float)w * S.tab.inv_scale[l]);
        L.h = cv_round((float)h * S.tab.inv_scale[l]);
        if (L.w < 2 * ORB_EDGE + 8 || L.h < 2 * ORB_EDGE + 8 || L.w > 4096 + 2 * ORB_BORDER || L.h > 4096 + 2 * ORB_BORDER)
            return ccm_fail(c, CCM_E_ARG, "level %d is %dx%d: unsupported image size", l, L.w, L.h);
        L.scale = S.tab.scale[l];
        L.kp_size = (float)(int)(31 * S.tab.scale[l]);
        L.quota = S.tab.nfeat[l];
        max_quota = std::max(max_quota, L.quota);
        L.spitch = (int)align_up(L.w, 64);
        L.splane = (long long)L.spitch * L.h;
        S.smap_off[l] = smap_bytes; smap_bytes += align_up((size_t)L.splane * nframes, 256);
        if (l > 0) {
            L.pitch = (int)align_up(L.w, 64);
            L.plane = (long long)L.pitch * L.h;
            S.pyr_off[l] = pyr_bytes; pyr_bytes += align_up((size_t)L.plane * nframes, 256);
            std::vector<int> xo, yo; std::vector<short> xa, ya;
            linear_tables(G.lv[l - 1].w, L.w, xo, xa);
            linear_tables(G.lv[l - 1].h, L.h, yo, ya);
            toff[l].xofs = tab_i.size(); tab_i.insert(tab_i.end(), xo.begin(), xo.end());
            toff[l].yofs = tab_i.size(); tab_i.insert(tab_i.end(), yo.begin(), yo.end());
            toff[l].xab = tab_s.size(); tab_s.insert(tab_s.end(), xa.begin(), xa.end());
            toff[l].yab = tab_s.size(); tab_s.insert(tab_s.end(), ya.begin(), ya.end());
        }
        const int minBX = ORB_BORDER, minBY = ORB_BORDER, maxBX = L.w - ORB_EDGE + 3, maxBY = L.h - ORB_EDGE + 3;
        const float width = (float)(maxBX - minBX), height = (float)(maxBY - minBY);
        const int nCols = (int)(width / 30.f), nRows = (int)(height / 30.f);
        L.bw = maxBX - minBX; L.bh = maxBY - minBY;
        L.cell_first = (int)S.cells.size();
        int key_cap = 0;
        if (nCols >= 1 && nRows >= 1) {
            const int wCell = (int)std::ceil(width / nCols), hCell = (int)std::ceil(height / nRows);
            for (int i = 0; i < nRows; i++) {
                const float iniY = (float)(minBY + i * hCell);
                float maxY = iniY + hCell + 6;
                if (iniY >= maxBY - 3) continue;
                if (maxY > maxBY) maxY = (float)maxBY;
                for (int j = 0; j < nCols; j++) {
                    const float iniX = (float)(minBX + j * wCell);
                    float maxX = iniX + wCell + 6;
                    if (iniX >= maxBX - 6) continue;
                    if (maxX > maxBX) maxX = (float)maxBX;
                    OrbCell cell{};
                    cell.level = (short)l; cell.x0 = (short)iniX; cell.y0 = (short)iniY;
                    cell.cw = (short)((int)maxX - (int)iniX); cell.ch = (short)((int)maxY - (int)iniY);
                    if (cell.cw > 65 || cell.ch > 65)
                        return ccm_fail(c, CCM_E_ARG, "FAST cell %dx%d exceeds the kernel tile", cell.cw, cell.ch);
                    const int rw = std::max(cell.cw - 6, 0), rh = std::max(cell.ch - 6, 0);
                    cell.slot_cap = ((rw + 1) / 2) * ((rh + 1) / 2);
                    cell.slot_first = slot_acc;
                    slot_acc += cell.slot_cap; key_cap += cell.slot_cap;
                    S.cells.push_back(cell);
                }
            }
        }
        L.ncells = (int)S.cells.size() - L.cell_first;
        L.roots = (int)std::round((float)(maxBX - minBX) / (maxBY - minBY));
        if (L.roots < 1 || L.roots > ORB_MAX_ROOTS)
            return ccm_fail(c, CCM_E_ARG, "level %d aspect ratio gives %d quadtree roots (1..%d supported)", l, L.roots, ORB_MAX_ROOTS);
        L.hx = (float)(maxBX - minBX) / L.roots;
        L.key_first = key_acc; L.key_cap = std::max(key_cap, 1); key_acc += L.key_cap;
        L.out_cap = std::max(L.quota + 4, 4 * L.roots);
        L.out_first = out_acc; out_acc += L.out_cap;
        L.tiles_x = (L.w + 63) / 64; L.tiles_y = (L.h + 63) / 64;
        L.tile_first = tile_acc; tile_acc += L.tiles_x * L.tiles_y;
    }
    S.bands.clear(); S.band_lds = 0;
    static const bool want_fused = !(getenv("CCM_ORB_FUSED") && atoi(getenv("CCM_ORB_FUSED")) == 0);
    S.fused = want_fused;
    static const int pcap = getenv("CCM_FC_PCAP") ? std::min(atoi(getenv("CCM_FC_PCAP")), 256) : 144;
    static const int scap = getenv("CCM_FC_SURV") ? atoi(getenv("CCM_FC_SURV")) : 3072;
    S.surv_cap = scap;
    for (size_t a = 0; a < S.cells.size();) {
        size_t b = a;
        const OrbCell& c0 = S.cells[a];
        const int xa = (c0.x0 - 4) & ~3;
        int pitch = 0;
        while (b < S.cells.size() && S.cells[b].level == c0.level && S.cells[b].y0 == c0.y0) {
            const int p2 = (int)align_up((size_t)(S.cells[b].x0 + S.cells[b].cw + 4 - xa), 16);
            if (b > a && (p2 > pcap || b - a >= ORB_BAND_CELLS)) break;
            pitch = p2; b++;
        }
        OrbBand band{};
        band.cell_first = (int)a; band.ncells = (int)(b - a); band.level = c0.level; band.xa = (short)xa; band.y0 = (short)c0.y0;
        band.pitch = (short)pitch; band.bh = (short)c0.ch;
        {
            const OrbCell& cl = S.cells[b - 1];
            const int PW = pitch / 4, PQ = std::max(pitch / 16, 1);
            band.c_lo = (short)(c0.x0 + 3 - xa); band.c_hi = (short)(cl.x0 + cl.cw - 3 - xa);
            band.dw_lo = (short)std::max(1, band.c_lo >> 2); band.dw_hi = (short)std::min(PW - 2, (band.c_hi - 1) >> 2);
            band.pw_inv = (1u << 20) / (unsigned)PW + 1u; band.pq_inv = (1u << 20) / (unsigned)PQ + 1u;
            band.w = G.lv[c0.level].w; band.h = G.lv[c0.level].h;
            for (size_t k = a; k < b; k++) {
                const OrbCell& ck = S.cells[k];
                band.clo[k - a] = (short)(ck.x0 + 3 - xa); band.cwd[k - a] = (short)(ck.cw - 6);
                band.slot_first[k - a] = ck.slot_first; band.slot_cap[k - a] = ck.slot_cap;
            }
        }
        for (size_t k = a; k < b; k++) if (S.cells[k].ch != c0.ch) S.fused = false;
        S.surv_cap = std::max(S.surv_cap, pitch);
        S.bands.push_back(band);
        a = b;
    }
    for (const OrbBand& b : S.bands) S.band_lds = std::max(S.band_lds, orb_fast_cells_lds(b.pitch, b.bh, S.surv_cap));
    for (const OrbBand& b : S.bands) if (b.pitch > 256) S.fused = false;
    if (S.band_lds > 60 * 1024) S.fused = false;
    G.ncells = (int)S.cells.size(); G.ntiles = tile_acc;
    G.slots_per_frame = std::max(slot_acc, 1); G.keys_per_frame = key_acc; G.out_per_frame = out_acc;
    int list_cap = 0;
    for (int l = 0; l < p->nlevels; l++) list_cap = std::max(list_cap, G.lv[l].out_cap);
    G.list_cap = (int)align_up(list_cap + 4, 16);
    if (orb_octree_lds_bytes(G.list_cap) > 150 * 1024)
        return ccm_fail(c, CCM_E_ARG, "nfeatures too large for the quadtree kernel's LDS (list cap %d)", G.list_cap);
    if (max_per_image < 1) return ccm_fail(c, CCM_E_ARG, "max_per_image must be positive");

    CCM_RESERVE(c, S.pyr, std::max<size_t>(pyr_bytes, 256));
    CCM_RESERVE(c, S.smap, smap_bytes);
    CCM_RESERVE(c, S.slots, (size_t)G.slots_per_frame * nframes * 4);
    CCM_RESERVE(c, S.cell_count, (size_t)std::max(G.ncells, 1) * nframes * 4);
    CCM_RESERVE(c, S.keysA, (size_t)G.keys_per_frame * nframes * 4);
    CCM_RESERVE(c, S.keysB, (size_t)G.keys_per_frame * nframes * 4);
    CCM_RESERVE(c, S.sel, (size_t)G.out_per_frame * nframes * 4);
    CCM_RESERVE(c, S.sel_count, (size_t)p->nlevels * nframes * 4);
    CCM_RESERVE(c, S.status, 256);
    CCM_RESERVE(c, S.kps, (size_t)nframes * max_per_image * sizeof(ccm_keypoint));
    CCM_RESERVE(c, S.desc, (size_t)nframes * max_per_image * 32);
    CCM_RESERVE(c, S.counts, (size_t)nframes * 4);
    const size_t tab_bytes = align_up(tab_i.size() * 4, 16) + tab_s.size() * 2;
    CCM_RESERVE(c, S.tables_dev, std::max<size_t>(tab_bytes, 16));
    CCM_RESERVE(c, S.cells_dev, std::max<size_t>(S.cells.size(), 1) * sizeof(OrbCell));
    CCM_RESERVE(c, S.bands_dev, std::max<size_t>(S.bands.size(), 1) * sizeof(OrbBand));
    CCM_RESERVE(c, S.geom_dev, sizeof(OrbGeom));
    char* tb = S.tables_dev.as<char>();
    const size_t s_base = align_up(tab_i.size() * 4, 16);
    for (int l = 0; l < p->nlevels; l++) {
        OrbLevel& L = G.lv[l];
        L.smap = S.smap.as<uint8_t>() + S.smap_off[l];
        if (l > 0) {
            L.img = S.pyr.as<uint8_t>() + S.pyr_off[l];
            L.xofs = reinterpret_cast<const int*>(tb) + toff[l].xofs;
            L.yofs = reinterpret_cast<const int*>(tb) + toff[l].yofs;
            L.xab = reinterpret_cast<const short*>(tb + s_base) + toff[l].xab;
            L.yab = reinterpret_cast<const short*>(tb + s_base) + toff[l].yab;
        }
    }
    if (!tab_i.empty()) CCM_HIP(c, hipMemcpyAsync(tb, tab_i.data(), tab_i.size() * 4, hipMemcpyHostToDevice, c->stream));
    if (!tab_s.empty()) CCM_HIP(c, hipMemcpyAsync(tb + s_base, tab_s.data(), tab_s.size() * 2, hipMemcpyHostToDevice, c->stream));
    if (!S.cells.empty())
        CCM_HIP(c, hipMemcpyAsync(S.cells_dev.p, S.cells.data(), S.cells.size() * sizeof(OrbCell), hipMemcpyHostToDevice, c->stream));
    for (OrbBand& b : S.bands) {
        const OrbLevel& L = G.lv[b.level];
        b.img = b.level > 0 ? L.img : nullptr; b.plane = L.plane; b.lpitch = L.pitch;
    }
    if (!S.bands.empty())
        CCM_HIP(c, hipMemcpyAsync(S.bands_dev.p, S.bands.data(), S.bands.size() * sizeof(OrbBand), hipMemcpyHostToDevice, c->stream));
    CCM_HIP(c, hipStreamSynchronize(c->stream));
    if (!S.pattern_up) { CCM_HIP(c, orb_upload_pattern()); S.pattern_up = true; }
    S.par = *p; S.w = w; S.h = h; S.nframes = nframes; S.max_per_image = max_per_image;
    S.valid = true;
    S.last_img = nullptr;
    return CCM_OK;
}

static int orb_run(ccm_ctx* c, const uint8_t* img_dev, int stride, size_t image_stride, int frame0 = 0, int nrun = -1)
{
    OrbState& S = *c->orb;
    OrbGeom& G = S.geom;
    G.lv[0].img = img_dev; G.lv[0].pitch = stride; G.lv[0].plane = (long long)image_stride;
    G.frame0 = frame0;
    if (nrun < 0) nrun = S.nframes - frame0;
    const OrbGeom& gd = G;
    const OrbCell* cd = S.cells_dev.as<OrbCell>();
    hipStream_t st = c->stream;
    if (frame0 == 0) CCM_HIP(c, hipMemsetAsync(S.status.p, 0, 4, st));
    for (int l = 1; l < G.nlevels; l++) { ProfScope ps(c, CCM_PROF_RESIZE); orb_launch_resize(st, gd, l, G.lv[l].w, G.lv[l].h, nrun); }
    if (S.fused && !S.bands.empty()) {
        ProfScope ps(c, CCM_PROF_FAST_SCORE);
        orb_launch_fast_cells(st, gd, cd, S.bands_dev.as<OrbBand>(), (int)S.bands.size(), nrun, S.band_lds, S.surv_cap, S.slots.as<unsigned>(), S.cell_count.as<int>());
    } else {
        { ProfScope ps(c, CCM_PROF_FAST_SCORE); orb_launch_score(st, gd, G.ntiles, nrun); }
        if (G.ncells > 0) { ProfScope ps(c, CCM_PROF_CELL_NMS); orb_launch_nms(st, gd, cd, G.ncells, nrun, S.slots.as<unsigned>(), S.cell_count.as<int>()); }
    }
    { ProfScope ps(c, CCM_PROF_OCTREE);
    orb_launch_octree(st, gd, cd, G.nlevels, nrun, G.list_cap, S.slots.as<unsigned>(), S.cell_count.as<int>(),
                      S.keysA.as<unsigned>(), S.keysB.as<unsigned>(), S.sel.as<unsigned>(), S.sel_count.as<int>(),
                      S.status.as<int>()); }
    { ProfScope ps(c, CCM_PROF_ORIENT_DESC);
    orb_launch_orient_desc(st, gd, G.out_per_frame, nrun, S.sel.as<unsigned>(), S.sel_count.as<int>(),
                           S.kps.as<ccm_keypoint>(), S.desc.as<uint8_t>(), S.counts.as<int>(), S.max_per_image,
                           S.status.as<int>()); }
    CCM_HIP(c, hipGetLastError());
    S.have_result = true;
    return CCM_OK;
}

static int orb_check_status(ccm_ctx* c)
{
    OrbState& S = *c->orb;
    int st = 0;
    CCM_HIP(c, hipMemcpyAsync(&st, S.status.p, 4, hipMemcpyDeviceToHost, c->stream));
    CCM_HIP(c, hipStreamSynchronize(c->stream));
    if (st & 8) return ccm_fail(c, CCM_E_CAPACITY, "an image produced more than max_per_image keypoints");
    if (st) return ccm_fail(c, CCM_E_DEVICE, "extractor kernel status 0x%x (1 key overflow, 2 quadtree guard, 4 list overflow)", st);
    return CCM_OK;
}

int orb_last_result(ccm_ctx* c, const ccm_keypoint** kps, const uint8_t** desc, const int32_t** counts, int* n_images, int* max_per_image,
                    int* nlevels)
{
    if (!c->orb || !c->orb->have_result) return ccm_fail(c, CCM_E_STATE, "no extraction on this context yet");
    const OrbState& S = *c->orb;
    *kps = S.kps.as<ccm_keypoint>(); *desc = S.desc.as<uint8_t>(); *counts = S.counts.as<int32_t>();
    *n_images = S.nframes; *max_per_image = S.max_per_image; *nlevels = S.par.nlevels;
    return CCM_OK;
}

extern "C" {

int ccm_orb_tables(const ccm_orb_params* p, float* scale, float* inv_scale, float* sigma2, float* inv_sigma2,
                   int32_t* features_per_level, int32_t* umax)
{
    OrbTables t;
    int rc = make_tables(p, &t);
    if (rc) return rc;
    for (int i = 0; i < p->nlevels; i++) {
        if (scale) scale[i] = t.scale[i];
        if (inv_scale) inv_scale[i] = t.inv_scale[i];
        if (sigma2) sigma2[i] = t.sigma2[i];
        if (inv_sigma2) inv_sigma2[i] = t.inv_sigma2[i];
        if (features_per_level) features_per_level[i] = t.nfeat[i];
    }
    if (umax) for (int i = 0; i < 16; i++) umax[i] = t.umax[i];
    return CCM_OK;
}

int ccm_orb_level_sizes(const ccm_orb_params* p, int w, int h, int32_t* level_w, int32_t* level_h)
{
    OrbTables t;
    int rc = make_tables(p, &t);
    if (rc) return rc;
    if (!level_w || !level_h) return CCM_E_ARG;
    for (int l = 0; l < p->nlevels; l++) {
        level_w[l] = cv_round((float)w * t.inv_scale[l]);
        level_h[l] = cv_round((float)h * t.inv_scale[l]);
    }
    return CCM_OK;
}

int ccm_orb_extract_dev(ccm_ctx* c, const ccm_orb_params* p, const uint8_t* img_dev, int w, int h, int stride,
                        size_t image_stride, int n_images, int max_per_image)
{
    RoctxRange roctx_("ccm_orb_extract_dev");
    return ccm_guard(c, "ccm_orb_extract_dev", [&]() -> int {
        if (!c || !p) return CCM_E_ARG;
        if (n_images == 0 || w == 0 || h == 0) return CCM_OK;
        if (!img_dev || w < 0 || h < 0 || n_images < 0 || stride < w || (n_images > 1 && image_stride < (size_t)stride * h))
            return ccm_fail(c, CCM_E_ARG, "bad image arguments");
        CCM_HIP(c, hipSetDevice(c->device));
        int rc = orb_prepare(c, p, w, h, n_images, max_per_image);
        if (rc) return rc;
        return orb_run(c, img_dev, stride, image_stride);
    });
}

int ccm_orb_fetch(ccm_ctx* c, ccm_keypoint* kps, uint8_t* desc, int32_t* counts)
{
    RoctxRange roctx_("ccm_orb_fetch");
    if (!c || !c->orb || !c->orb->have_result) return c ? ccm_fail(c, CCM_E_STATE, "no extraction to fetch") : CCM_E_ARG;
    OrbState& S = *c->orb;
    int rc = orb_check_status(c);
    if (rc) return rc;
    if (kps) CCM_HIP(c, hipMemcpyAsync(kps, S.kps.p, (size_t)S.nframes * S.max_per_image * sizeof(ccm_keypoint), hipMemcpyDeviceToHost, c->stream));
    if (desc) CCM_HIP(c, hipMemcpyAsync(desc, S.desc.p, (size_t)S.nframes * S.max_per_image * 32, hipMemcpyDeviceToHost, c->stream));
    if (counts) CCM_HIP(c, hipMemcpyAsync(counts, S.counts.p, (size_t)S.nframes * 4, hipMemcpyDeviceToHost, c->stream));
    CCM_HIP(c, hipStreamSynchronize(c->stream));
    return CCM_OK;
}

int ccm_orb_extract(ccm_ctx* c, const ccm_orb_params* p, const uint8_t* img, int w, int h, int stride,
                    size_t image_stride, int n_images, ccm_keypoint* kps, uint8_t* desc, int32_t* counts,
                    int max_per_image)
{
    RoctxRange roctx_("ccm_orb_extract");
    return ccm_guard(c, "ccm_orb_extract", [&]() -> int {
        if (!c || !p) return CCM_E_ARG;
        if (n_images == 0 || w == 0 || h == 0) return CCM_OK;
        if (!img || w < 0 || h < 0 || n_images < 0 || stride < w) return ccm_fail(c, CCM_E_ARG, "bad image arguments");
        CCM_HIP(c, hipSetDevice(c->device));
        if (!c->orb) c->orb = new OrbState();
        OrbState& S = *c->orb;
        static const bool force_2d = getenv("CCM_ORB_UPLOAD_2D") && atoi(getenv("CCM_ORB_UPLOAD_2D")) != 0;
        static const int chunk_frames = getenv("CCM_ORB_CHUNK") ? std::max(1, atoi(getenv("CCM_ORB_CHUNK"))) : 64;
        const int n_chunks = n_images >= 2 * chunk_frames ? (n_images + chunk_frames - 1) / chunk_frames : 1;
        const bool linear = !force_2d && n_chunks > 1 && stride % 16 == 0 && image_stride % 16 == 0 && image_stride >= (size_t)stride * h;
        const int pitch = linear ? stride : (int)align_up(w, 64);
        const size_t plane = linear ? image_stride : (size_t)pitch * h;
        CCM_RESERVE(c, S.img0, plane * n_images + 64);
        int rc = orb_prepare(c, p, w, h, n_images, max_per_image);
        if (rc) return rc;
        if (n_chunks > 1 && !S.copy_stream) {
            if (!(S.copy_stream = ccm_aux_stream(c, 0))) return ccm_fail(c, CCM_E_DEVICE, "hipStreamCreate failed");
            CCM_HIP(c, hipEventCreateWithFlags(&S.copy_done, hipEventDisableTiming));
        }
        const bool contiguous = n_images == 1 || image_stride == (size_t)stride * h;
        auto page_locked = [](const void* q) {
            if (!q) return true;
            hipPointerAttribute_t a{};
            if (hipPointerGetAttributes(&a, q) != hipSuccess) { (void)hipGetLastError(); return false; }
            return a.type == hipMemoryTypeHost;
        };
        const bool stream_down = n_chunks > 1 && (kps || desc || counts) && page_locked(kps) && page_locked(desc) && page_locked(counts);
        if (stream_down && !S.down_stream) {
            if (!(S.down_stream = ccm_aux_stream(c, 1))) return ccm_fail(c, CCM_E_DEVICE, "hipStreamCreate failed");
            CCM_HIP(c, hipEventCreateWithFlags(&S.chunk_done, hipEventDisableTiming));
        }
        for (int ck = 0; ck < n_chunks; ck++) {
            const int f0 = (int)((long long)n_images * ck / n_chunks), f1 = (int)((long long)n_images * (ck + 1) / n_chunks);
            hipStream_t up = n_chunks > 1 ? S.copy_stream : c->stream;
            if (linear) {
                const size_t bytes = f1 < n_images ? plane * (f1 - f0) : plane * (f1 - 1 - f0) + (size_t)stride * (h - 1) + w;
                CCM_HIP(c, hipMemcpyAsync(S.img0.as<char>() + plane * f0, img + image_stride * f0, bytes, hipMemcpyHostToDevice, up));
            } else if (contiguous) {
                CCM_HIP(c, hipMemcpy2DAsync(S.img0.as<char>() + plane * f0, pitch, img + image_stride * f0, stride, w, (size_t)h * (f1 - f0),
                                            hipMemcpyHostToDevice, up));
            } else {
                for (int i = f0; i < f1; i++)
                    CCM_HIP(c, hipMemcpy2DAsync(S.img0.as<char>() + plane * i, pitch, img + image_stride * i, stride, w, h, hipMemcpyHostToDevice, up));
            }
            if (n_chunks > 1) {
                CCM_HIP(c, hipEventRecord(S.copy_done, up));
                CCM_HIP(c, hipStreamWaitEvent(c->stream, S.copy_done, 0));
            }
// ... 67 lines not shown
```

### motioncheck_ccm_slam_amd/csrc/orb_kernels.hip

```cpp
#include <hip/hip_runtime.h>
#include "orb_types.h"
#include "../../include/ccm_orb_pattern.h"
#include "../../include/ccm_sincos.h"
#include "../../include/ccm_hot.h"

#define WAVE 64

typedef unsigned short fc_us2 __attribute__((ext_vector_type(2)));
__device__ __forceinline__ fc_us2 fc_pk(unsigned x) { return __builtin_bit_cast(fc_us2, x); }
__device__ __forceinline__ unsigned fc_u(fc_us2 x) { return __builtin_bit_cast(unsigned, x); }

__device__ __forceinline__ int lane_id() { return threadIdx.x & 63; }
__device__ __forceinline__ unsigned long long lanemask_lt() { return (1ull << lane_id()) - 1ull; }

__device__ __forceinline__ void xcd_work_item(int on, int& x, int& y)
{
    x = (int)blockIdx.x; y = (int)blockIdx.y;
    if (!on) return;
    const unsigned gx = gridDim.x, total = gx * gridDim.y;
    const unsigned lin = blockIdx.y * gx + blockIdx.x;
    unsigned w;
    if (on == 1) {
        const unsigned xcd = lin & 7u, q = total >> 3, rem = total & 7u;
        w = xcd * q + (xcd < rem ? xcd : rem) + (lin >> 3);
    } else {
        const unsigned C = (unsigned)on, span = 8u * C;
        const unsigned full = total - total % span;
        if (lin >= full) w = lin;
        else {
            const unsigned xcd = lin & 7u, j = lin >> 3;
            const unsigned super = j / C, within = j - super * C;
            w = (super * 8u + xcd) * C + within;
        }
    }
    unsigned q = (unsigned)((float)w * __frcp_rn((float)gx));
    if (q * gx > w) q--; else if ((q + 1u) * gx <= w) q++;
    y = (int)q; x = (int)(w - q * gx);
}

__device__ __forceinline__ int wave_incl_scan(int v)
{
    const int lane = lane_id();
#pragma unroll
    for (int d = 1; d < 64; d <<= 1) {
        int y = __shfl_up(v, d, 64);
        if (lane >= d) v += y;
    }
    return v;
}
__device__ __forceinline__ int wave_sum(int v)
{
#pragma unroll
    for (int d = 32; d >= 1; d >>= 1) v += __shfl_xor(v, d, 64);
    return v;
}
__device__ __forceinline__ void wave_sum2_dpp(int& x, int& y)
{
#define WS2_STEP(ctrl, rows) { const int tx = __builtin_amdgcn_update_dpp(0, x, ctrl, rows, 0xf, false); \
                               const int ty = __builtin_amdgcn_update_dpp(0, y, ctrl, rows, 0xf, false); x += tx; y += ty; }
    WS2_STEP(0xb1, 0xf)
    WS2_STEP(0x4e, 0xf)
    WS2_STEP(0x141, 0xf)
    WS2_STEP(0x140, 0xf)
    WS2_STEP(0x142, 0xa)
    WS2_STEP(0x143, 0xc)
#undef WS2_STEP
    x = __builtin_amdgcn_readlane(x, 63);
    y = __builtin_amdgcn_readlane(y, 63);
}

#ifndef RS_ROWS
#define RS_ROWS 8
#endif
__global__ __launch_bounds__(256) void k_pyr_resize(const OrbGeom g, int level)
{
    const OrbLevel& D = g.lv[level];
    const OrbLevel& S = g.lv[level - 1];
    const int lane = threadIdx.x & 63;
    const int x4 = (blockIdx.x * 64 + lane) * 4;
    const int yb = (blockIdx.y * 4 + __builtin_amdgcn_readfirstlane(threadIdx.x >> 6)) * RS_ROWS;
    const int f = blockIdx.z + g.frame0;
    if (yb >= D.h) return;
    const uint8_t* src = S.img + (long long)f * S.plane;
    uint8_t* dstp = const_cast<uint8_t*>(D.img) + (long long)f * D.plane;
    int yo; unsigned ybb;
    {
        const int y = min(yb + (lane & (RS_ROWS - 1)), D.h - 1);
        yo = D.yofs[y];
        __builtin_memcpy(&ybb, D.yab + 2 * y, 4);
    }
    const uint8_t* r0p[RS_ROWS]; const uint8_t* r1p[RS_ROWS]; unsigned b0[RS_ROWS], b1[RS_ROWS];
#pragma unroll
    for (int r = 0; r < RS_ROWS; r++) {
        const int sy0 = __builtin_amdgcn_readlane(yo, r);
        const unsigned bb = (unsigned)__builtin_amdgcn_readlane((int)ybb, r);
        r0p[r] = src + (long long)sy0 * S.pitch;
        r1p[r] = src + (long long)min(sy0 + 1, S.h - 1) * S.pitch;
        b0[r] = bb & 0xFFFFu; b1[r] = bb >> 16;
    }
    if (x4 >= D.w) return;
    {
        int sxs[4]; unsigned abw[4];
        if (x4 + 3 < D.w) {
            int4 so; uint4 ab;
            __builtin_memcpy(&so, D.xofs + x4, 16);
            __builtin_memcpy(&ab, D.xab + 2 * x4, 16);
            sxs[0] = so.x; sxs[1] = so.y; sxs[2] = so.z; sxs[3] = so.w;
            abw[0] = ab.x; abw[1] = ab.y; abw[2] = ab.z; abw[3] = ab.w;
        } else {
#pragma unroll
            for (int i = 0; i < 4; i++) {
                const int x = min(x4 + i, D.w - 1);
                sxs[i] = D.xofs[x];
                __builtin_memcpy(&abw[i], D.xab + 2 * x, 4);
            }
        }
        const int base = min(sxs[0], S.w - 8);
        const int ba = min(base & ~3, S.pitch - 12);
        if (S.w >= 8 && S.pitch >= 12 && sxs[3] - base <= 7) {
            uint2 q0[RS_ROWS], q1[RS_ROWS];
            const unsigned sh = (unsigned)(base - ba);
            const bool sh4 = sh > 3u;
#pragma unroll
            for (int r = 0; r < RS_ROWS; r++) {
                const unsigned* p0 = reinterpret_cast<const unsigned*>(r0p[r] + (unsigned)ba);
                const unsigned* p1 = reinterpret_cast<const unsigned*>(r1p[r] + (unsigned)ba);
                const unsigned d00 = p0[0], d01 = p0[1], d02 = p0[2], d10 = p1[0], d11 = p1[1], d12 = p1[2];
                const unsigned l0 = sh4 ? d01 : d00, m0 = sh4 ? d02 : d01, l1 = sh4 ? d11 : d10, m1 = sh4 ? d12 : d11;
                q0[r].x = __builtin_amdgcn_alignbyte(m0, l0, sh); q0[r].y = __builtin_amdgcn_alignbyte(d02, m0, sh);
                q1[r].x = __builtin_amdgcn_alignbyte(m1, l1, sh); q1[r].y = __builtin_amdgcn_alignbyte(d12, m1, sh);
            }
            unsigned sel[4];
#pragma unroll
            for (int i = 0; i < 4; i++) {
                const unsigned o = (unsigned)(sxs[i] - base);
                sel[i] = 0x0c000c00u + o + (min(o + 1u, 7u) << 16);
            }
#pragma unroll
            for (int r = 0; r < RS_ROWS; r++) {
                unsigned out = 0;
#pragma unroll
                for (int i = 0; i < 4; i++) {
                    const unsigned h0 = __builtin_amdgcn_udot2(fc_pk(__builtin_amdgcn_perm(q0[r].y, q0[r].x, sel[i])), fc_pk(abw[i]), 0u, false);
                    const unsigned h1 = __builtin_amdgcn_udot2(fc_pk(__builtin_amdgcn_perm(q1[r].y, q1[r].x, sel[i])), fc_pk(abw[i]), 0u, false);
                    const unsigned v = ((__umul24(b0[r], h0 >> 4) >> 16) + (__umul24(b1[r], h1 >> 4) >> 16) + 2u) >> 2;
                    out |= v << (8 * i);
                }
                if (yb + r < D.h) *reinterpret_cast<unsigned*>(dstp + (long long)(yb + r) * D.pitch + (unsigned)x4) = out;
            }
            return;
        }
    }
    for (int r = 0; r < RS_ROWS && yb + r < D.h; r++) {
        unsigned out = 0;
#pragma unroll
        for (int i = 0; i < 4; i++) {
            const int x = min(x4 + i, D.w - 1);
            const int sx0 = D.xofs[x];
            const int sx1 = min(sx0 + 1, S.w - 1);
            const int a0 = D.xab[2 * x], a1 = D.xab[2 * x + 1];
            const int h0 = r0p[r][sx0] * a0 + r0p[r][sx1] * a1;
            const int h1 = r1p[r][sx0] * a0 + r1p[r][sx1] * a1;
            const int v = ((((int)b0[r] * (h0 >> 4)) >> 16) + (((int)b1[r] * (h1 >> 4)) >> 16) + 2) >> 2;
            out |= (unsigned)(v & 255) << (8 * i);
        }
        *reinterpret_cast<unsigned*>(dstp + (long long)(yb + r) * D.pitch + (unsigned)x4) = out;
    }
}

__host__ __device__ inline int fast_score16(int v, const int* r)
{
    int d[16];
#pragma unroll
    for (int k = 0; k < 16; k++) d[k] = v - r[k];
    int lo3[16], hi3[16];
#pragma unroll
    for (int k = 0; k < 16; k++) {
        const int a = d[k], b = d[(k + 1) & 15], c = d[(k + 2) & 15];
        lo3[k] = min(a, min(b, c));
        hi3[k] = max(a, max(b, c));
    }
    int A = -256, B = 256;
#pragma unroll
    for (int k = 0; k < 16; k++) {
        A = max(A, min(lo3[k], min(lo3[(k + 3) & 15], lo3[(k + 6) & 15])));
        B = min(B, max(hi3[k], max(hi3[(k + 3) & 15], hi3[(k + 6) & 15])));
    }
    return max(A, -B) - 1;
}

#define ST_W 64
#define ST_H 64
#define ST_LW 72
#define ST_LH (ST_H + 6)

__global__ __launch_bounds__(256) void k_fast_score(const OrbGeom g)
{
    __shared__ __attribute__((aligned(16))) uint8_t tile[ST_LH][ST_LW];
    __shared__ __attribute__((aligned(16))) uint8_t outt[ST_H][ST_W];
    __shared__ unsigned short surv[ST_W * ST_H];
    __shared__ int nsurv;
    int t = blockIdx.x, level = 0;
    for (int l = 1; l < g.nlevels; l++)
        if (t >= g.lv[l].tile_first) level = l;
    const OrbLevel& L = g.lv[level];
    t -= L.tile_first;
    const int tx0 = (t % L.tiles_x) * ST_W, ty0 = (t / L.tiles_x) * ST_H;
    const int f = blockIdx.y + g.frame0;
    const uint8_t* img = L.img + (long long)f * L.plane;
    if (threadIdx.x == 0) nsurv = 0;
    for (int i = threadIdx.x; i < ST_H * ST_W / 4; i += 256) reinterpret_cast<unsigned*>(&outt[0][0])[i] = 0u;
    const bool dword_ok = ((reinterpret_cast<uintptr_t>(img) | (uintptr_t)L.pitch) & 3) == 0 && L.pitch >= ((L.w + 3) & ~3);
    if (dword_ok) {
        const int wmax = ((L.w - 1) & ~3);
        for (int i = threadIdx.x; i < ST_LH * (ST_LW / 4); i += 256) {
            const int ly = i / (ST_LW / 4), lx = i - ly * (ST_LW / 4);
            const int gy = min(max(ty0 + ly - 3, 0), L.h - 1);
            const int gx = min(max(tx0 + 4 * lx - 4, 0), wmax);
            reinterpret_cast<unsigned*>(&tile[ly][0])[lx] = *reinterpret_cast<const unsigned*>(img + (long long)gy * L.pitch + gx);
        }
    } else {
        for (int i = threadIdx.x; i < ST_LH * ST_LW; i += 256) {
            const int ly = i / ST_LW, lx = i - ly * ST_LW;
            const int gy = min(max(ty0 + ly - 3, 0), L.h - 1);
            const int gx = min(max(tx0 + lx - 4, 0), L.w - 1);
            tile[ly][lx] = img[(long long)gy * L.pitch + gx];
        }
    }
// ... 31 lines not shown
                    int base = 0;
                    if (lane_id() == 0) base = atomicAdd(&nsurv, __popcll(m));
                    base = __shfl(base, 0, 64);
                    if (keep) surv[base + __popcll(m & lanemask_lt())] = (unsigned short)(py * ST_W + px + i);
                }
            }
        }
    }
    __syncthreads();
    const int ns = nsurv;
    for (int si = threadIdx.x; si < ns; si += 256) {
        const int pos = surv[si];
        const int cy = (pos >> 6) + 3, cx = (pos & 63) + 4;
        const int v = tile[cy][cx];
        int r[16];
        r[0] = tile[cy + 3][cx];      r[1] = tile[cy + 3][cx + 1];  r[2] = tile[cy + 2][cx + 2];
        r[3] = tile[cy + 1][cx + 3];  r[4] = tile[cy][cx + 3];      r[5] = tile[cy - 1][cx + 3];
        r[6] = tile[cy - 2][cx + 2];  r[7] = tile[cy - 3][cx + 1];  r[8] = tile[cy - 3][cx];
        r[9] = tile[cy - 3][cx - 1];  r[10] = tile[cy - 2][cx - 2]; r[11] = tile[cy - 1][cx - 3];
        r[12] = tile[cy][cx - 3];     r[13] = tile[cy + 1][cx - 3]; r[14] = tile[cy + 2][cx - 2];
        r[15] = tile[cy + 3][cx - 1];
        const int sc = fast_score16(v, r);
        if (sc >= t_lo && sc > 0) outt[pos >> 6][pos & 63] = (uint8_t)sc;
    }
    __syncthreads();
    for (int py = threadIdx.x >> 4; py < ST_H; py += 16) {
        const int gy = ty0 + py;
        if (gy < L.h && tx0 + px < L.spitch)
            *reinterpret_cast<unsigned*>(L.smap + (long long)f * L.splane + (long long)gy * L.spitch + tx0 + px) =
                reinterpret_cast<const unsigned*>(&outt[py][0])[px >> 2];
    }
}

#define NMS_PITCH 72
#define NMS_ROWS 62
#define NMS_WAVE_LDS (NMS_PITCH * NMS_ROWS)
__global__ __launch_bounds__(256) void k_cell_nms(const OrbGeom g, const OrbCell* __restrict__ cells,
                                                  unsigned* __restrict__ slots, int* __restrict__ cell_count)
{
    __shared__ __attribute__((aligned(16))) uint8_t lds[4][NMS_WAVE_LDS];
    const int wv = threadIdx.x >> 6, lane = lane_id();
    const int ci = blockIdx.x * 4 + wv;
    if (ci >= g.ncells) return;
    const int f = blockIdx.y + g.frame0;
    const OrbCell c = cells[ci];
    const OrbLevel& L = g.lv[c.level];
    const int rx0 = c.x0 + 3, ry0 = c.y0 + 3, rw = c.cw - 6, rh = c.ch - 6;
    int* count_out = cell_count + (long long)f * g.ncells + ci;
    if (rw <= 0 || rh <= 0) { if (lane == 0) *count_out = 0; return; }
    uint8_t* T = lds[wv];
    const uint8_t* sm = L.smap + (long long)f * L.splane;
    for (int i = lane; i < NMS_PITCH / 4; i += 64) {
        reinterpret_cast<unsigned*>(T)[i] = 0u;
        reinterpret_cast<unsigned*>(T + (rh + 1) * NMS_PITCH)[i] = 0u;
    }
    const int lx = (lane & 15) * 4, lrow = lane >> 4;
    bool any = false;
    {
        unsigned v[15];
#pragma unroll
        for (int it = 0; it < 15; it++) {
            const int yy = 4 * it + lrow;
            v[it] = 0;
            if (yy < rh && lx < rw) __builtin_memcpy(&v[it], sm + (long long)(ry0 + yy) * L.spitch + rx0 + lx, 4);
        }
        const int valid = rw - lx;
        const unsigned keep_mask = valid >= 4 ? 0xFFFFFFFFu : (valid <= 0 ? 0u : (1u << (8 * valid)) - 1u);
#pragma unroll
        for (int it = 0; it < 15; it++) {
            const int yy = 4 * it + lrow;
            if (yy < rh) {
                const unsigned w = v[it] & keep_mask;
                *reinterpret_cast<unsigned*>(T + (yy + 1) * NMS_PITCH + 4 + lx) = w;
                if ((lane & 15) == 0) *reinterpret_cast<unsigned*>(T + (yy + 1) * NMS_PITCH) = 0u;
                any |= w != 0u;
            }
        }
    }
    if (__ballot(any) == 0ull) { if (lane == 0) *count_out = 0; return; }
    __builtin_amdgcn_s_waitcnt(0xc07f);
    __builtin_amdgcn_wave_barrier();
    unsigned* out = slots + (long long)f * g.slots_per_frame + c.slot_first;
    const int relx = rx0 - ORB_BORDER, rely = ry0 - ORB_BORDER;
    int n = 0;
    const int rpi = rw <= 32 ? 2 : 1;
    const int xx = rpi == 2 ? (lane & 31) : lane, yoff = rpi == 2 ? (lane >> 5) : 0;
    for (int attempt = 0; attempt < 2 && n == 0; attempt++) {
        const int th = attempt == 0 ? g.ini_th : g.min_th;
        for (int y0 = 0; y0 < rh; y0 += rpi) {
            const int yy = y0 + yoff;
            bool keep = false;
            int s = 0;
            const uint8_t* p = &T[(min(yy, rh - 1) + 1) * NMS_PITCH + 4 + xx];
            if (yy < rh && xx < rw) s = p[0];
            if (__ballot(s >= th && s > 0) == 0ull) continue;
            {
                if (s >= th && s > 0) {
#define NB(o) ((int)p[o] >= th ? (int)p[o] : 0)
                    keep = s > NB(-1) && s > NB(1) &&
                           s > NB(-NMS_PITCH - 1) && s > NB(-NMS_PITCH) && s > NB(-NMS_PITCH + 1) &&
                           s > NB(NMS_PITCH - 1) && s > NB(NMS_PITCH) && s > NB(NMS_PITCH + 1);
#undef NB
                }
            }
            const unsigned long long m = __ballot(keep);
            if (keep) {
                const int pos = n + __popcll(m & lanemask_lt());
                if (pos < c.slot_cap)
                    out[pos] = ((unsigned)s << 24) | ((unsigned)(rely + yy) << 12) | (unsigned)(relx + xx);
            }
            n += __popcll(m);
        }
    }
    if (lane == 0) *count_out = n;
}

#ifndef FC_NZ
#define FC_NZ 1024
#endif
#ifndef FC_KEPT
#define FC_KEPT 480
#endif
#define FC_CELLS 32
#ifndef FC_TPB
#define FC_TPB 256
#endif
__host__ __device__ inline int fc_wave_cap(int surv_cap) { (void)surv_cap; return 320; }
__host__ __device__ inline size_t fc_lds_bytes(int pitch, int bh, int surv_cap)
{
    return 2 * (size_t)pitch * bh + (size_t)fc_wave_cap(surv_cap) * (FC_TPB / 64) * 2 + 32 + FC_NZ * 2 + FC_KEPT * 4 + FC_CELLS * 16 + 64 * 8 + 256 + 64;
}


__device__ __forceinline__ int fc_mbcnt(unsigned long long m, int base)
{
    return (int)__builtin_amdgcn_mbcnt_hi((unsigned)(m >> 32), __builtin_amdgcn_mbcnt_lo((unsigned)m, (unsigned)base));
}
#ifdef FC_STAMPS
#define FC_STAMP_SLOTS 8
#define FC_STAMP_WGS (1 << 17)
__device__ unsigned long long fc_stamps[FC_STAMP_WGS * FC_STAMP_SLOTS];
#define FC_STAMP(k) do { if (threadIdx.x == 0) { const unsigned wg__ = blockIdx.y * gridDim.x + blockIdx.x; if (wg__ < FC_STAMP_WGS) fc_stamps[wg__ * FC_STAMP_SLOTS + (k)] = __builtin_amdgcn_s_memtime(); } } while (0)
extern "C" int ccm_debug_fc_stamps(unsigned long long* out, int n_wgs)
{
    return hipMemcpyFromSymbol(out, HIP_SYMBOL(fc_stamps), (size_t)n_wgs * FC_STAMP_SLOTS * 8, 0, hipMemcpyDeviceToHost) == hipSuccess ? 0 : -1;
}
#else
#define FC_STAMP(k) do { } while (0)
#endif
template <class T>
__device__ __forceinline__ int sel4(int ci, const T (&a)[4]) { return ci == 0 ? (int)a[0] : ci == 1 ? (int)a[1] : ci == 2 ? (int)a[2] : (int)a[3]; }
template <bool PACKED>
__global__ __launch_bounds__(FC_TPB) __attribute__((amdgpu_waves_per_eu(8, 8))) void k_fast_cells(const OrbGeom g, const OrbCell* __restrict__ cells, const OrbBand* __restrict__ bands,
                                                    unsigned* __restrict__ slots, int* __restrict__ cell_count, int unused_, int abl, int xcd_on)
{
    extern __shared__ __attribute__((aligned(16))) uint8_t fc_smem[];
    int wx, wy;
    xcd_work_item(xcd_on, wx, wy);
    FC_STAMP(0);
    const OrbBand B = bands[wx];
#ifdef FC_STAMPS
    asm volatile("s_waitcnt lgkmcnt(0)" ::: "memory");
#endif
    FC_STAMP(6);
    int bclo[4], bcwd[4], bsfirst[4], bscap[4];
#pragma unroll
    for (int i = 0; i < 4; i++) {
        bclo[i] = B.clo[i]; bcwd[i] = B.cwd[i]; bsfirst[i] = B.slot_first[i]; bscap[i] = B.slot_cap[i];
        asm volatile("" : "+s"(bclo[i]), "+s"(bcwd[i]), "+s"(bsfirst[i]), "+s"(bscap[i]));
    }
    int bxa = B.xa, by0 = B.y0, bncells = B.ncells, bcfirst = B.cell_first;
    asm volatile("" : "+s"(bxa), "+s"(by0), "+s"(bncells), "+s"(bcfirst));
    const int f = wy + g.frame0, tid = threadIdx.x, lane = lane_id(), wv = tid >> 6;
    const bool lvl0 = B.level == 0;
    const uint8_t* const Limg = lvl0 ? g.lv[0].img : B.img;
    const long long Lplane = lvl0 ? g.lv[0].plane : B.plane;
    const int Lpitch = lvl0 ? g.lv[0].pitch : B.lpitch, Lw = B.w, Lh = B.h;
    const int P = B.pitch, bh = B.bh, PW = P >> 2;
    uint8_t* T = fc_smem;
    uint8_t* S = fc_smem + (size_t)P * bh;
    constexpr int NW = FC_TPB / 64;
    const int WCAP = fc_wave_cap(0);
    unsigned short* surv = reinterpret_cast<unsigned short*>(S + (size_t)P * bh);
    int* nsurv = reinterpret_cast<int*>(surv + NW * WCAP);
    unsigned short* nz = reinterpret_cast<unsigned short*>(nsurv + 8);
    unsigned* kept = reinterpret_cast<unsigned*>(nz + FC_NZ);
    int* cell_hi = reinterpret_cast<int*>(kept + FC_KEPT);
    int* cell_n = cell_hi + FC_CELLS;
    int* cell_k = cell_n + FC_CELLS;
    uint2* colmask = reinterpret_cast<uint2*>(cell_k + FC_CELLS + FC_CELLS);
    uint8_t* colcell = reinterpret_cast<uint8_t*>(colmask + 64);
    if (tid < FC_CELLS) { cell_hi[tid] = 0; cell_n[tid] = 0; cell_k[tid] = 0; }
    int* l_clo = reinterpret_cast<int*>(colcell + 256); int* l_cwd = l_clo + 4; int* l_sfirst = l_cwd + 4; int* l_scap = l_sfirst + 4;
    if (tid < 4) { l_clo[tid] = sel4(tid, bclo); l_cwd[tid] = sel4(tid, bcwd); l_sfirst[tid] = sel4(tid, bsfirst); l_scap[tid] = sel4(tid, bscap); }
    if (tid == 0) { nsurv[1] = 0; nsurv[2] = 0; }
    const uint8_t* img = Limg + (long long)f * Lplane;
    const bool dword_ok = ((reinterpret_cast<uintptr_t>(img) | (uintptr_t)Lpitch) & 3) == 0 && Lpitch >= ((Lw + 3) & ~3);
    const unsigned pw_inv = B.pw_inv;
#ifdef FC_STAMPS
    asm volatile("s_waitcnt lgkmcnt(0)" ::: "memory");
#endif
    FC_STAMP(5);
    if (dword_ok && (P & 15) == 0) {
        const int wmax = ((Lw - 1) & ~3);
        const int PQ = P >> 4;
        const unsigned pq_inv = B.pq_inv;
        for (int i = tid; i < bh * PQ; i += FC_TPB) {
            const int ly = (int)(((unsigned)i * pq_inv) >> 20), lq = i - ly * PQ;
            const int gy = min(B.y0 + ly, Lh - 1), gx = B.xa + 16 * lq;
            const uint8_t* rowp = img + (long long)gy * Lpitch;
            uint4 v;
            if (gx + 12 <= wmax) __builtin_memcpy(&v, rowp + gx, 16);
            else {
                v.x = *reinterpret_cast<const unsigned*>(rowp + min(gx, wmax));
                v.y = *reinterpret_cast<const unsigned*>(rowp + min(gx + 4, wmax));
                v.z = *reinterpret_cast<const unsigned*>(rowp + min(gx + 8, wmax));
                v.w = *reinterpret_cast<const unsigned*>(rowp + min(gx + 12, wmax));
            }
            reinterpret_cast<uint4*>(T)[i] = v;
            reinterpret_cast<uint4*>(S)[i] = make_uint4(0u, 0u, 0u, 0u);
        }
    } else if (dword_ok) {
        const int wmax = ((Lw - 1) & ~3);
        for (int i = tid; i < bh * PW; i += FC_TPB) {
            const int ly = (int)(((unsigned)i * pw_inv) >> 20), lx = i - ly * PW;
            const int gy = min(B.y0 + ly, Lh - 1), gx = min(B.xa + 4 * lx, wmax);
            reinterpret_cast<unsigned*>(T)[i] = *reinterpret_cast<const unsigned*>(img + (long long)gy * Lpitch + gx);
            reinterpret_cast<unsigned*>(S)[i] = 0u;
        }
    } else {
        for (int i = tid; i < bh * P; i += FC_TPB) {
            const int ly = i / P, lx = i - ly * P;
            const int gy = min(B.y0 + ly, Lh - 1), gx = min(B.xa + lx, Lw - 1);
            T[i] = img[(long long)gy * Lpitch + gx];
            S[i] = 0;
        }
    }
#ifdef FC_STAMPS
    asm volatile("s_waitcnt vmcnt(0)" ::: "memory");
#endif
    FC_STAMP(7);
    const int c_lo = B.c_lo, c_hi = B.c_hi;
    const int t_lo = min(g.ini_th, g.min_th);
    const int dw_lo = B.dw_lo, dw_hi = B.dw_hi;
    if (tid < PW) {
        unsigned mk[4];
        for (int i = 0; i < 4; i++) mk[i] = (4 * tid + i >= c_lo && 4 * tid + i < c_hi) ? 0xFFFFu : 0u;
        colmask[tid] = make_uint2(mk[0] | (mk[2] << 16), mk[1] | (mk[3] << 16));
    }
    __syncthreads();
    FC_STAMP(1);
    if (abl == 1) return;
    if (tid < P) {
        int ci = 255;
#pragma unroll
        for (int i = 0; i < ORB_BAND_CELLS; i++) if (i < bncells && tid >= bclo[i] && tid < bclo[i] + bcwd[i]) ci = i;
        colcell[tid] = (uint8_t)ci;
    }
    unsigned short* wsurv = surv + wv * WCAP;
    auto score_at = [&](int pos) {
        const uint8_t* c = T + pos;
        const int v = c[0];
        int r[16];
        r[0] = c[3 * P];      r[1] = c[3 * P + 1];  r[2] = c[2 * P + 2];  r[3] = c[P + 3];
        r[4] = c[3];          r[5] = c[-P + 3];     r[6] = c[-2 * P + 2]; r[7] = c[-3 * P + 1];
        r[8] = c[-3 * P];     r[9] = c[-3 * P - 1]; r[10] = c[-2 * P - 2]; r[11] = c[-P - 3];
        r[12] = c[-3];        r[13] = c[P - 3];     r[14] = c[2 * P - 2]; r[15] = c[3 * P - 1];
        const int sc = fast_score16(v, r);
        if (sc >= t_lo && sc > 0) {
            S[pos] = (uint8_t)sc;
            const int q = atomicAdd(nsurv + 1, 1);
            if (q < FC_NZ) nz[q] = (unsigned short)pos;
        }
    };
    {
        int wcnt = 0;
        const int items = (bh - 6) * PW;
        constexpr int r0 = 3;
        for (int it0 = wv * 64; it0 < items; it0 += FC_TPB) {
            const int it = it0 + lane;
            const int rr = (int)(((unsigned)it * pw_inv) >> 20);
            const int row = r0 + rr, dw = it - rr * PW;
            const int px = 4 * dw;
            unsigned keep4 = 0;
            unsigned kk0 = 0, kk1 = 0;
            if (!PACKED && it < items && px + 3 >= c_lo && px < c_hi && dw >= 1 && dw + 1 < PW) {
                const unsigned* crow = reinterpret_cast<const unsigned*>(T + row * P) + dw;
                const unsigned c0 = crow[-1], c1 = crow[0], c2 = crow[1];
                const unsigned nn = reinterpret_cast<const unsigned*>(T + (row + 3) * P)[dw];
                const unsigned ss = reinterpret_cast<const unsigned*>(T + (row - 3) * P)[dw];
                const unsigned long long lo = ((unsigned long long)c1 << 32) | c0, hi = ((unsigned long long)c2 << 32) | c1;
#pragma unroll
                for (int i = 0; i < 4; i++) {
                    const int col = px + i;
                    if (col < c_lo || col >= c_hi) continue;
                    const int v = (int)((c1 >> (8 * i)) & 0xFF);
                    const int n = (int)((nn >> (8 * i)) & 0xFF), s2 = (int)((ss >> (8 * i)) & 0xFF);
                    const int w = (int)((lo >> (8 * (i + 1))) & 0xFF);
                    const int e = (int)((hi >> (8 * (i + 3))) & 0xFF);
                    const bool keep = !((abs(v - n) <= t_lo && abs(v - s2) <= t_lo) || (abs(v - e) <= t_lo && abs(v - w) <= t_lo));
                    keep4 |= keep ? (1u << i) : 0u;
                }
            }
            if (PACKED && it < items && dw >= dw_lo && dw <= dw_hi) {
                const unsigned* crow = reinterpret_cast<const unsigned*>(T + r0 * P) + it;
                const unsigned c0 = crow[-1], c1 = crow[0], c2 = crow[1];
                const unsigned nn = crow[3 * PW], ss = crow[-3 * PW];
                const unsigned ww = __builtin_amdgcn_alignbyte(c1, c0, 1);
                const unsigned ee = __builtin_amdgcn_alignbyte(c2, c1, 3);
// ... 551 lines not shown
            prow[i] = v;
        }
    }
}
template <int ITEMS>
__global__ __launch_bounds__(64 * OD_WAVES) __attribute__((amdgpu_waves_per_eu(8, 8))) void k_orient_desc(const OrbGeom g, const unsigned* __restrict__ sel,
                                                     const int* __restrict__ sel_count,
                                                     ccm_keypoint* __restrict__ kps, uint8_t* __restrict__ desc,
                                                     int* __restrict__ counts, int max_per_image, int* __restrict__ status, int xcd_on)
{
    extern __shared__ __attribute__((aligned(16))) uint8_t od_pad[];
    __shared__ __attribute__((aligned(16))) uint8_t lds[OD_WAVES][OD_WAVE_LDS_PAD];
    __shared__ unsigned wone[16][11], wu[16][11], pat[256];
    const int wv = __builtin_amdgcn_readfirstlane((int)(threadIdx.x >> 6)), lane = lane_id();
    int wx, wy;
    xcd_work_item(xcd_on, wx, wy);
    const int f = wy + g.frame0;
    const int* sc = sel_count + (long long)f * g.nlevels;
    const int slot = (wx * ITEMS + min(lane, ITEMS - 1)) * OD_WAVES + wv;
    const unsigned key_l = slot < g.out_per_frame ? sel[(long long)f * g.out_per_frame + slot] : 0u;
    for (int i = threadIdx.x; i < 256; i += 64 * OD_WAVES) pat[i] = *reinterpret_cast<const unsigned*>(c_pattern + 4 * i);
    for (int i = threadIdx.x; i < 16 * 11; i += 64 * OD_WAVES) {
        const int av = i / 11, k = i - av * 11;
        const int lim = g.umax[av];
        unsigned a = 0, b = 0;
        for (int j = 0; j < 4; j++) {
            const int u = 4 * k + j - ORB_PATCH_R;
            if (u >= -lim && u <= lim) { a |= 1u << (8 * j); b |= (unsigned)(u + 16) << (8 * j); }
        }
        wone[av][k] = a; wu[av][k] = b;
    }
    int level_l = 0, first_l = 0;
    for (int l = 1; l < g.nlevels; l++) if (slot >= g.lv[l].out_first) { level_l = l; first_l = g.lv[l].out_first; }
    int row_l = slot - first_l, tot = 0, cnt_l = 0;
    for (int l = 0; l < g.nlevels; l++) { const int c = sc[l]; if (l < level_l) row_l += c; if (l == level_l) cnt_l = c; tot += c; }
    if (wx == 0 && wv == 0 && lane == 0) {
        counts[f] = min(tot, max_per_image);
        if (tot > max_per_image) atomicOr(status, 8);
    }
    if (wx == 0) {
        const long long r0 = (long long)f * max_per_image + min(tot, max_per_image);
        const int npad = max_per_image - min(tot, max_per_image);
        unsigned* kz = reinterpret_cast<unsigned*>(kps + r0);
        for (int i = threadIdx.x; i < npad * 7; i += 64 * OD_WAVES) kz[i] = 0u;
        uint4* dz = reinterpret_cast<uint4*>(desc + r0 * 32);
        for (int i = threadIdx.x; i < npad * 2; i += 64 * OD_WAVES) dz[i] = make_uint4(0u, 0u, 0u, 0u);
    }
    const bool valid_l = lane < ITEMS && slot < g.out_per_frame && slot - first_l < cnt_l && row_l < max_per_image;
    unsigned long long todo = __ballot(valid_l);
    __syncthreads();
    if (todo == 0) return;

    uint8_t* wl = lds[wv];
    const float factorPI = (float)(3.14159265358979323846 / 180.f);
    auto item_of = [&](int j, OdItem& it, int& level, int& score, int& row) {
        const unsigned key = (unsigned)__builtin_amdgcn_readlane((int)key_l, j);
        level = __builtin_amdgcn_readlane(level_l, j); row = __builtin_amdgcn_readlane(row_l, j);
        const OrbLevel& L = g.lv[level];
        it.img = L.img + (long long)f * L.plane; it.pitch = L.pitch; it.w = L.w; it.h = L.h;
        it.cx = (int)(key & 0xFFFu) + ORB_BORDER; it.cy = (int)((key >> 12) & 0xFFFu) + ORB_BORDER;
        score = (int)(key >> 24);
    };
    unsigned prow[11];
    OdItem it; int level, score, row;
    {
        const int j = __builtin_ctzll(todo); todo &= todo - 1;
        item_of(j, it, level, score, row);
        od_load_patch(it, lane, prow);
    }
    for (;;) {
        int m10 = 0, m01 = 0;
        {
            const int v = lane - ORB_PATCH_R, av = v < 0 ? -v : v;
            if (av <= ORB_HALF_PATCH) {
                unsigned s1 = 0, su = 0;
#pragma unroll
                for (int i = 1; i < 10; i++) {
                    s1 = __builtin_amdgcn_udot4(prow[i], wone[av][i], s1, false);
                    su = __builtin_amdgcn_udot4(prow[i], wu[av][i], su, false);
                }
                m10 = (int)su - 16 * (int)s1;
                m01 = v * (int)s1;
            }
        }
        wave_sum2_dpp(m10, m01);
        const float angle = fast_atan2_deg((float)m01, (float)m10);

        __builtin_amdgcn_s_waitcnt(0xc07f);
        if (lane < ORB_PATCH_D) {
            const unsigned Q0 = 18u | (34u << 8) | (49u << 16) | (55u << 24), Q1 = 49u | (34u << 8) | (18u << 16);
#pragma unroll
            for (int x = 0; x < ORB_BLUR_D; x++) {
                const int kk = x >> 2, sh = x & 3;
                const unsigned w0 = sh ? __builtin_amdgcn_alignbyte(prow[kk + 1], prow[kk], sh) : prow[kk];
                const unsigned w1 = sh ? __builtin_amdgcn_alignbyte(prow[kk + 2 > 10 ? 10 : kk + 2], prow[kk + 1], sh) : prow[kk + 1];
                const unsigned h = __builtin_amdgcn_udot4(w1, Q1, __builtin_amdgcn_udot4(w0, Q0, 0u, false), false);
                *reinterpret_cast<unsigned short*>(wl + x * OD_HT_PITCH + 2 * lane) = (unsigned short)h;
            }
        }
        const bool more = todo != 0;
        const int cx = it.cx, cy = it.cy, level_c = level, score_c = score, row_c = row;
        if (more) {
            const int j = __builtin_ctzll(todo); todo &= todo - 1;
            item_of(j, it, level, score, row);
            od_load_patch(it, lane, prow);
        }
        __builtin_amdgcn_s_waitcnt(0xc07f);
        __builtin_amdgcn_wave_barrier();

        float a, b;
        ccm_sincosf(angle * factorPI, &b, &a);
        uint8_t* drow = desc + ((long long)f * max_per_image + row_c) * 32;
        const uint8_t* ctr = wl + 18 * OD_HT_PITCH + 4 * 9;
        unsigned long long mybits = 0;
#pragma unroll
        for (int r0 = 0; r0 < 4; r0 += OD_BRIEF_BATCH) {
            OdTaps tp[OD_BRIEF_BATCH][2];
#pragma unroll
            for (int q = 0; q < OD_BRIEF_BATCH; q++) {
                const unsigned pr = pat[(r0 + q) * 64 + lane];
                const float x0 = (float)(signed char)(pr & 255u), y0 = (float)(signed char)((pr >> 8) & 255u);
                const float x1 = (float)(signed char)((pr >> 16) & 255u), y1 = (float)(signed char)(pr >> 24);
                od_gather(ctr, __float2int_rn(x0 * a - y0 * b), __float2int_rn(x0 * b + y0 * a), tp[q][0]);
                od_gather(ctr, __float2int_rn(x1 * a - y1 * b), __float2int_rn(x1 * b + y1 * a), tp[q][1]);
            }
            if (OD_BRIEF_BATCH > 1) __builtin_amdgcn_sched_barrier(0);
#pragma unroll
            for (int q = 0; q < OD_BRIEF_BATCH; q++) {
                const unsigned long long bits = __ballot(od_blur_at(tp[q][0]) < od_blur_at(tp[q][1]));
                if (lane == r0 + q) mybits = bits;
            }
        }
        if (lane < 4) *reinterpret_cast<unsigned long long*>(drow + 8 * lane) = mybits;
        if (lane == 0) {
            const OrbLevel& L = g.lv[level_c];
            ccm_keypoint kp;
            kp.x = (float)cx; kp.y = (float)cy;
            if (level_c != 0) { kp.x *= L.scale; kp.y *= L.scale; }
            kp.size = L.kp_size; kp.angle = angle; kp.response = (float)score_c;
            kp.octave = level_c; kp.class_id = -1;
            kps[(long long)f * max_per_image + row_c] = kp;
        }
        if (!more) break;
    }
}

extern "C" hipError_t orb_upload_pattern()
{
    return hipMemcpyToSymbol(HIP_SYMBOL(c_pattern), ccm_orb_pattern, 1024);
}

size_t orb_octree_lds_bytes(int list_cap) { return (size_t)list_cap * OCT_NODE_LDS + 64 + 4 * (size_t)OCT_LDS_KEYS + 8 * (size_t)list_cap; }

void orb_launch_resize(hipStream_t s, const OrbGeom& g_dev, int level, int dw, int dh, int nframes)
{
    dim3 grid((dw + 255) / 256, (dh + 4 * RS_ROWS - 1) / (4 * RS_ROWS), nframes);
    hipLaunchKernelGGL(k_pyr_resize, grid, dim3(256), 0, s, g_dev, level);
}
void orb_launch_score(hipStream_t s, const OrbGeom& g_dev, int ntiles, int nframes)
{
    hipLaunchKernelGGL(k_fast_score, dim3(ntiles, nframes), dim3(256), 0, s, g_dev);
}
void orb_launch_nms(hipStream_t s, const OrbGeom& g_dev, const OrbCell* cells, int ncells, int nframes,
                    unsigned* slots, int* cell_count)
{
    hipLaunchKernelGGL(k_cell_nms, dim3((ncells + 3) / 4, nframes), dim3(256), 0, s, g_dev, cells, slots, cell_count);
}
void orb_launch_fast_cells(hipStream_t s, const OrbGeom& g_dev, const OrbCell* cells, const OrbBand* bands, int nbands, int nframes,
                           size_t lds_bytes, int surv_cap, unsigned* slots, int* cell_count)
{
    static const bool packed = !(getenv("CCM_FC_PACKED") && atoi(getenv("CCM_FC_PACKED")) == 0);
    static const int abl = getenv("CCM_FC_ABL") ? atoi(getenv("CCM_FC_ABL")) : 0;
    static const int xcd_on = getenv("CCM_ORB_XCD_FC") ? atoi(getenv("CCM_ORB_XCD_FC")) : (getenv("CCM_ORB_XCD") ? atoi(getenv("CCM_ORB_XCD")) : 0);
    static const size_t lds_min = getenv("CCM_FC_LDS_MIN") ? (size_t)atol(getenv("CCM_FC_LDS_MIN")) : 0;
    if (lds_bytes < lds_min) lds_bytes = lds_min;
    (void)surv_cap;
    if (packed) hipLaunchKernelGGL(k_fast_cells<true>, dim3(nbands, nframes), dim3(FC_TPB), lds_bytes, s, g_dev, cells, bands, slots, cell_count, 0, abl, xcd_on);
    else hipLaunchKernelGGL(k_fast_cells<false>, dim3(nbands, nframes), dim3(FC_TPB), lds_bytes, s, g_dev, cells, bands, slots, cell_count, 0, abl, xcd_on);
}
size_t orb_fast_cells_lds(int pitch, int bh, int surv_cap) { return fc_lds_bytes(pitch, bh, surv_cap); }
void orb_launch_octree(hipStream_t s, const OrbGeom& g_dev, const OrbCell* cells, int nlevels, int nframes, int list_cap,
                       const unsigned* slots, const int* cell_count, unsigned* keysA, unsigned* keysB,
                       unsigned* out, int* out_count, int* status)
{
    static const int key_parallel = !(getenv("CCM_OCT_REG_KEYS") && atoi(getenv("CCM_OCT_REG_KEYS")) == 0);
    hipLaunchKernelGGL(k_octree, dim3(nframes, nlevels), dim3(64 * OCT_WAVES), orb_octree_lds_bytes(list_cap), s,
                       g_dev, cells, slots, cell_count, keysA, keysB, out, out_count, status, key_parallel);
}
void orb_launch_orient_desc(hipStream_t s, const OrbGeom& g_dev, int out_per_frame, int nframes, const unsigned* sel,
                            const int* sel_count, ccm_keypoint* kps, uint8_t* desc, int* counts, int max_per_image,
                            int* status)
{
    static const int xcd_on = getenv("CCM_ORB_XCD_OD") ? atoi(getenv("CCM_ORB_XCD_OD")) : (getenv("CCM_ORB_XCD") ? atoi(getenv("CCM_ORB_XCD")) : 1);
    static const size_t lds_pad = getenv("CCM_OD_LDS_PAD") ? (size_t)atol(getenv("CCM_OD_LDS_PAD")) : 0;
    if ((long long)out_per_frame * nframes < 4 * 8192)
        hipLaunchKernelGGL(k_orient_desc<1>, dim3((out_per_frame + OD_WAVES - 1) / OD_WAVES, nframes), dim3(64 * OD_WAVES), lds_pad, s,
                           g_dev, sel, sel_count, kps, desc, counts, max_per_image, status, xcd_on);
    else
        hipLaunchKernelGGL(k_orient_desc<OD_ITEMS>, dim3((out_per_frame + OD_WAVES * OD_ITEMS - 1) / (OD_WAVES * OD_ITEMS), nframes), dim3(64 * OD_WAVES), lds_pad, s,
                           g_dev, sel, sel_count, kps, desc, counts, max_per_image, status, xcd_on);
}
```

Before: 281.7 Mfeatures/s.

## Add FP4 scaled-MFMA Hamming matcher and fold status clear into resize kernel

Adds an FP4 variant of the MFMA Hamming brute-force kernel. Descriptor bits are expanded to FP4 nibbles and fed to the scaled f8f6f4 32x32x64 MFMA with float accumulators, so each tile needs 4 k-steps instead of 8. The min/second-min keys are carried as floats. Variants 3 and 5 now dispatch to the FP4 path while variant 4 keeps the int8 path; a debug entry point tests one FP4 tile. Separately, the status memset is removed and the first resize or fast_cells kernel zeroes the status word, saving one async memset call. This relies on packed index/distance keys staying exactly representable in float, which bounds the key range.

```diff
diff --git a/include/ccm_hot.h b/include/ccm_hot.h
--- a/include/ccm_hot.h
+++ b/include/ccm_hot.h
@@ -81,6 +81,7 @@
 int ccm_hamming_match(ccm_ctx*, const uint8_t* q, int nq, const uint8_t* t, int nt, int n_pairs,
                       const int32_t* nq_n, const int32_t* nt_n,
                       int32_t* best_idx, int32_t* best_dist, int32_t* second_dist);
+int ccm_debug_fp4_tile(ccm_ctx*, const uint8_t* a, const uint8_t* b, const float* row_c, float* out);
 int ccm_hamming_match_dev(ccm_ctx*, const uint8_t* q_dev, int nq, size_t q_pair_stride,
                           const uint8_t* t_dev, int nt, size_t t_pair_stride, int n_pairs,
                           const int32_t* nq_n_dev, const int32_t* nt_n_dev,
diff --git a/motioncheck_ccm_slam_amd/_lib.py b/motioncheck_ccm_slam_amd/_lib.py
--- a/motioncheck_ccm_slam_amd/_lib.py
+++ b/motioncheck_ccm_slam_amd/_lib.py
@@ -21,7 +21,7 @@
     "ccm_host_register", "ccm_host_unregister", "ccm_profile_enable", "ccm_profile_read",
     "ccm_orb_tables", "ccm_orb_level_sizes", "ccm_orb_extract", "ccm_orb_extract_dev", "ccm_orb_fetch",
     "ccm_orb_result_dev", "ccm_orb_debug_level", "ccm_orb_debug_candidates",
-    "ccm_descriptor_distance", "ccm_hamming_match", "ccm_hamming_match_dev", "ccm_ratio_test", "ccm_match_bow",
+    "ccm_descriptor_distance", "ccm_hamming_match", "ccm_hamming_match_dev", "ccm_debug_fp4_tile", "ccm_ratio_test", "ccm_match_bow",
     "ccm_window_candidates", "ccm_search_by_projection", "ccm_search_by_projection_frame", "ccm_search_for_initialization", "ccm_fuse_select", "ccm_fuse_select_batch", "ccm_search_by_sim3", "ccm_search_by_projection_sim3", "ccm_search_by_projection_sim3_batch",
     "ccm_search_for_triangulation", "ccm_voc_create", "ccm_voc_destroy", "ccm_voc_words", "ccm_voc_transform", "ccm_voc_transform_dev",
     "ccm_bow_vector", "ccm_bow_score_l1", "ccm_distinctive_descriptors", "ccm_optimize_sim3", "ccm_optimize_essential_graph", "ccm_correct_map_points",
@@ -146,6 +146,7 @@
     lib.ccm_hamming_match.argtypes = [vp, vp, C.c_int, vp, C.c_int, C.c_int, vp, vp, vp, vp, vp]
     lib.ccm_hamming_match_dev.argtypes = [vp, vp, C.c_int, C.c_size_t, vp, C.c_int, C.c_size_t, C.c_int,
                                           vp, vp, vp, vp, vp]
+    lib.ccm_debug_fp4_tile.argtypes = [vp, vp, vp, vp, vp]
     lib.ccm_ratio_test.argtypes = [C.c_int, C.c_int, C.c_float, C.c_int, C.c_int]
     lib.ccm_match_bow.argtypes = [vp, C.POINTER(BowOptions), vp, vp, vp, vp, C.c_int, vp, vp, vp, vp, C.c_int, vp]
     lib.ccm_window_candidates.argtypes = [vp, C.POINTER(FrameGrid), C.c_int, vp, vp, vp, vp, vp, vp, C.c_int, vp, vp, vp]
diff --git a/motioncheck_ccm_slam_amd/csrc/match_host.cpp b/motioncheck_ccm_slam_amd/csrc/match_host.cpp
--- a/motioncheck_ccm_slam_amd/csrc/match_host.cpp
+++ b/motioncheck_ccm_slam_amd/csrc/match_host.cpp
@@ -10,6 +10,7 @@
                      unsigned* part_best, int* part_second, int* bi, int* bd, int* sd);
 void match_launch_ranges(hipStream_t, const uint8_t* d1, const uint8_t* d2, const int* order2, const int* start,
                          const int* len, const long long* off, int n1, unsigned short* dist);
+void match_launch_fp4_tile(hipStream_t, const unsigned* a, const unsigned* b, const float* c, float* out);
 struct BowDev {
     int n_groups, n1;
     const int* ga; const int* gae; const int* gb; const int* gbe;
@@ -116,6 +117,24 @@
         CCM_HIP(c, hipMemcpyAsync(best_idx, M.bi.p, ob, hipMemcpyDeviceToHost, c->stream));
         CCM_HIP(c, hipMemcpyAsync(best_dist, M.bd.p, ob, hipMemcpyDeviceToHost, c->stream));
         CCM_HIP(c, hipMemcpyAsync(second_dist, M.sd.p, ob, hipMemcpyDeviceToHost, c->stream));
+        CCM_HIP(c, hipStreamSynchronize(c->stream));
+        return CCM_OK;
+    });
+}
+
+int ccm_debug_fp4_tile(ccm_ctx* c, const uint8_t* a, const uint8_t* b, const float* row_c, float* out)
+{
+    return ccm_guard(c, "ccm_debug_fp4_tile", [&]() -> int {
+        if (!c) return CCM_E_ARG;
+        if (!a || !b || !row_c || !out) return ccm_fail(c, CCM_E_ARG, "bad FP4 tile arguments");
+        CCM_HIP(c, hipSetDevice(c->device));
+        MatchState& M = *match_state(c);
+        int rc;
+        if ((rc = ccm_upload(c, M.q, a, 1024, c->stream)) || (rc = ccm_upload(c, M.t, b, 1024, c->stream)) || (rc = ccm_upload(c, M.bd, row_c, 128, c->stream))) return rc;
+        CCM_RESERVE(c, M.sd, 4096);
+        match_launch_fp4_tile(c->stream, M.q.as<unsigned>(), M.t.as<unsigned>(), M.bd.as<float>(), M.sd.as<float>());
+        CCM_HIP(c, hipGetLastError());
+        CCM_HIP(c, hipMemcpyAsync(out, M.sd.p, 4096, hipMemcpyDeviceToHost, c->stream));
         CCM_HIP(c, hipStreamSynchronize(c->stream));
         return CCM_OK;
     });
diff --git a/motioncheck_ccm_slam_amd/csrc/match_kernels.hip b/motioncheck_ccm_slam_amd/csrc/match_kernels.hip
--- a/motioncheck_ccm_slam_amd/csrc/match_kernels.hip
+++ b/motioncheck_ccm_slam_amd/csrc/match_kernels.hip
@@ -85,7 +85,9 @@
 }
 
 typedef int hm_v4i __attribute__((ext_vector_type(4)));
+typedef int hm_v8i __attribute__((ext_vector_type(8)));
 typedef int hm_v16i __attribute__((ext_vector_type(16)));
+typedef float hm_v16f __attribute__((ext_vector_type(16)));
 #ifndef HM_CB
 #define HM_CB 2
 #endif
@@ -100,15 +102,27 @@
 #endif
 #define HM_QW (32 * HM_CB)
 #define HM_TPB (64 * HM_WAVES)
-#define HM_SENT 0x3FFFFFFF
 #define HM_MAX_NT 2048
-
 #define HM_BIAS 4352
 #define HM_IDX_BITS 11
-__device__ __forceinline__ int hm_med3(int a, int b, int c)
-{
-    return __float_as_int(__builtin_amdgcn_fmed3f(__int_as_float(a), __int_as_float(b), __int_as_float(c)));
-}
+#define HM_SCALE 0x85858585
+
+template <bool FP4> struct HmForm;
+template <> struct HmForm<false> {
+    typedef int key; typedef hm_v16i acc;
+    static constexpr int KS = 8;
+    static __device__ __forceinline__ int sent() { return 0x3FFFFFFF; }
+};
+template <> struct HmForm<true> {
+    typedef float key; typedef hm_v16f acc;
+    static constexpr int KS = 4;
+    static __device__ __forceinline__ float sent() { return 16777216.0f; }
+};
+
+__device__ __forceinline__ float hm_med3(float a, float b, float c) { return __builtin_amdgcn_fmed3f(a, b, c); }
+__device__ __forceinline__ int hm_med3(int a, int b, int c) { return __float_as_int(hm_med3(__int_as_float(a), __int_as_float(b), __int_as_float(c))); }
+__device__ __forceinline__ float hm_min(float a, float b) { return __builtin_amdgcn_fmed3f(a, b, 0.0f); }
+__device__ __forceinline__ int hm_min(int a, int b) { return min(a, b); }
 
 __device__ __forceinline__ hm_v4i hm_expand16(unsigned hw, int shift)
 {
@@ -118,14 +132,42 @@
     v.z = (int)(__umul24((hs >> 8) & nm, 0x204081u) & bm); v.w = (int)(__umul24((hs >> 12) & nm, 0x204081u) & bm);
     return v;
 }
-
+__device__ __forceinline__ int hm_nibbles8(unsigned b, unsigned one)
+{
+    unsigned x = (b | (b << 12)) & 0x000F000Fu;
+    x = (x | (x << 6)) & 0x03030303u;
+    x = (x | (x << 3)) & 0x11111111u;
+    return (int)(x * one);
+}
+__device__ __forceinline__ hm_v4i hm_expand32_fp4(unsigned w, unsigned one)
+{
+    hm_v4i v;
+    v.x = hm_nibbles8(w & 255u, one); v.y = hm_nibbles8((w >> 8) & 255u, one);
+    v.z = hm_nibbles8((w >> 16) & 255u, one); v.w = hm_nibbles8(w >> 24, one);
+    return v;
+}
+__device__ __forceinline__ hm_v16i hm_mfma(const hm_v4i& a, const hm_v4i& b, const hm_v16i& c)
+{
+    return __builtin_amdgcn_mfma_i32_32x32x32_i8(a, b, c, 0, 0, 0);
+}
+__device__ __forceinline__ hm_v16f hm_mfma(const hm_v4i& a, const hm_v4i& b, const hm_v16f& c)
+{
+    const hm_v8i a8 = { a.x, a.y, a.z, a.w, 0, 0, 0, 0 }, b8 = { b.x, b.y, b.z, b.w, 0, 0, 0, 0 };
+    return __builtin_amdgcn_mfma_scale_f32_32x32x64_f8f6f4(a8, b8, c, 4, 4, 0, (int)HM_SCALE, 0, (int)HM_SCALE);
+}
+
+template <bool FP4>
 __global__ __launch_bounds__(HM_TPB, HM_WG_PER_CU * HM_TPB / 256) void k_hamming_mfma(
     const uint8_t* __restrict__ q, long long q_pair_bytes, const uint8_t* __restrict__ t, long long t_pair_bytes,
     int nq, int nt, const int* __restrict__ nq_n, const int* __restrict__ nt_n, int q_blocks,
     int* __restrict__ best_idx, int* __restrict__ best_dist, int* __restrict__ second_dist)
 {
-    __shared__ hm_v4i frag[2][HM_TT * 8][64];
-    __shared__ __attribute__((aligned(16))) int wall[HM_MAX_NT];
+    typedef HmForm<FP4> F;
+    typedef typename F::key key_t;
+    typedef typename F::acc acc_t;
+    constexpr int KS = F::KS;
+    __shared__ hm_v4i frag[2][HM_TT * KS][64];
+    __shared__ __attribute__((aligned(16))) key_t wall[HM_MAX_NT];
     const int pair = blockIdx.x / q_blocks, qblk = blockIdx.x - pair * q_blocks;
     const int tid = threadIdx.x, lane = tid & 63, wv = tid >> 6, h = lane >> 5, r = lane & 31;
     const int nqp = nq_n ? min(max(nq_n[pair], 0), nq) : nq;
@@ -141,75 +183,86 @@
         return;
     }
 
-    hm_v4i bq[HM_CB][8];
+    hm_v4i bq[HM_CB][KS];
     int pa[HM_CB];
 #pragma unroll
     for (int cb = 0; cb < HM_CB; cb++) {
         const int qi = q0 + 32 * cb + r;
-        unsigned d[8];
-        int pc = 0;
-#pragma unroll
-        for (int s = 0; s < 8; s++) { d[s] = qi < nqp ? qp[8 * (long long)qi + s] : 0u; pc += __popc(d[s]); }
-        pa[cb] = pc;
-#pragma unroll
-        for (int s = 0; s < 8; s++) bq[cb][s] = hm_expand16((d[s] >> (16 * h)) & 0xFFFFu, 7);
-    }
-    int m1[HM_CB], m2[HM_CB];
-#pragma unroll
-    for (int cb = 0; cb < HM_CB; cb++) { m1[cb] = HM_SENT; m2[cb] = HM_SENT; }
-
-    constexpr int HM_FPT = (512 * HM_TT + HM_TPB - 1) / HM_TPB;
+        if constexpr (FP4) {
+            const uint4 d = qi < nqp ? reinterpret_cast<const uint4*>(qp + 8 * (long long)qi)[h] : make_uint4(0, 0, 0, 0);
+            const int pc = __popc(d.x) + __popc(d.y) + __popc(d.z) + __popc(d.w);
+            pa[cb] = pc + __shfl_xor(pc, 32, 64);
+            bq[cb][0] = hm_expand32_fp4(d.x, 10u); bq[cb][1] = hm_expand32_fp4(d.y, 10u);
+            bq[cb][2] = hm_expand32_fp4(d.z, 10u); bq[cb][3] = hm_expand32_fp4(d.w, 10u);
+        } else {
+            unsigned d[8];
+            int pc = 0;
+#pragma unroll
+            for (int s = 0; s < 8; s++) { d[s] = qi < nqp ? qp[8 * (long long)qi + s] : 0u; pc += __popc(d[s]); }
+            pa[cb] = pc;
+#pragma unroll
+            for (int s = 0; s < 8; s++) bq[cb][s] = hm_expand16((d[s] >> (16 * h)) & 0xFFFFu, 7);
+        }
+    }
+    key_t m1[HM_CB], m2[HM_CB];
+#pragma unroll
+    for (int cb = 0; cb < HM_CB; cb++) { m1[cb] = F::sent(); m2[cb] = F::sent(); }
+
+    constexpr int FR = 64 * KS, HM_FPT = (FR * HM_TT + HM_TPB - 1) / HM_TPB;
     struct Raw { unsigned v[HM_FPT]; };
     auto fetch = [&](int group) {
         Raw x;
 #pragma unroll
         for (int j = 0; j < HM_FPT; j++) {
-            const int fi = tid + j * HM_TPB, sub = fi >> 9, fw = fi & 511;
+            const int fi = tid + j * HM_TPB, sub = fi / FR, fw = fi % FR;
             const int tr = (group * HM_TT + sub) * 32 + (fw & 31);
-            x.v[j] = (fi < 512 * HM_TT && tr < ntp) ? tp[8 * (long long)tr + ((fw >> 5) & 7)] : 0u;
+            x.v[j] = (fi < FR * HM_TT && tr < ntp) ? tp[8 * (long long)tr + ((fw >> 5) & 7)] : 0u;
         }
         return x;
     };
     auto stage = [&](const Raw& x, int buf) {
 #pragma unroll
         for (int j = 0; j < HM_FPT; j++) {
-            const int fi = tid + j * HM_TPB, sub = fi >> 9, fw = fi & 511;
-            if (fi < 512 * HM_TT) frag[buf][8 * sub + ((fw >> 5) & 7)][32 * (fw >> 8) + (fw & 31)] = hm_expand16((x.v[j] >> (16 * (fw >> 8))) & 0xFFFFu, 5);
+            const int fi = tid + j * HM_TPB, sub = fi / FR, fw = fi % FR;
+            if (fi >= FR * HM_TT) continue;
+            if constexpr (FP4) frag[buf][KS * sub + ((fw >> 5) & 3)][32 * (fw >> 7) + (fw & 31)] = hm_expand32_fp4(x.v[j], 2u);
+            else frag[buf][KS * sub + ((fw >> 5) & 7)][32 * (fw >> 8) + (fw & 31)] = hm_expand16((x.v[j] >> (16 * (fw >> 8))) & 0xFFFFu, 5);
         }
     };
     for (int tr = tid; tr < ((ntp + 31) & ~31); tr += HM_TPB) {
-        int w = HM_SENT;
+        key_t w = F::sent();
         if (tr < ntp) {
             const uint4* d = reinterpret_cast<const uint4*>(tp + 8 * (long long)tr);
             const uint4 d0 = d[0], d1 = d[1];
             const int pb = __popc(d0.x) + __popc(d0.y) + __popc(d0.z) + __popc(d0.w) + __popc(d1.x) + __popc(d1.y) + __popc(d1.z) + __popc(d1.w);
-            w = ((pb + HM_BIAS) << HM_IDX_BITS) | tr;
+            w = (key_t)(((pb + HM_BIAS) << HM_IDX_BITS) | tr);
         }
         wall[tr] = w;
     }
     const int ntiles = (ntp + 31) >> 5;
     const bool wave_live = q0 < nqp;
-    auto mma = [&](int tile, int buf, int sub, hm_v16i (&acc)[HM_CB]) {
-        hm_v16i wc;
+    auto mma = [&](int tile, int buf, int sub, acc_t (&acc)[HM_CB]) {
+        typedef key_t key4 __attribute__((ext_vector_type(4)));
+        acc_t wc;
 #pragma unroll
         for (int g = 0; g < 4; g++) {
-            const hm_v4i w4 = *reinterpret_cast<const hm_v4i*>(&wall[32 * tile + 8 * g + 4 * h]);
+            const key4 w4 = *reinterpret_cast<const key4*>(&wall[32 * tile + 8 * g + 4 * h]);
             wc[4 * g] = w4.x; wc[4 * g + 1] = w4.y; wc[4 * g + 2] = w4.z; wc[4 * g + 3] = w4.w;
         }
 #pragma unroll
-        for (int s = 0; s < 8; s++) {
-            const hm_v4i a = frag[buf][8 * sub + s][lane];
-#pragma unroll
-            for (int cb = 0; cb < HM_CB; cb++) acc[cb] = __builtin_amdgcn_mfma_i32_32x32x32_i8(a, bq[cb][s], s == 0 ? wc : acc[cb], 0, 0, 0);
+        for (int s = 0; s < KS; s++) {
+            const hm_v4i a = frag[buf][KS * sub + s][lane];
+#pragma unroll
+            for (int cb = 0; cb < HM_CB; cb++) acc[cb] = hm_mfma(a, bq[cb][s], s == 0 ? wc : acc[cb]);
         }
     };
-    auto fold = [&](const hm_v16i (&acc)[HM_CB]) {
+    auto fold = [&](const acc_t (&acc)[HM_CB]) {
 #pragma unroll
         for (int i = 0; i < 16; i++)
 #pragma unroll
             for (int cb = 0; cb < HM_CB; cb++) {
-                const int kx = acc[cb][i];
-                m2[cb] = hm_med3(m1[cb], m2[cb], kx); m1[cb] = min(m1[cb], kx);
+                const key_t kx = acc[cb][i];
+                m2[cb] = hm_med3(m1[cb], m2[cb], kx); m1[cb] = hm_min(m1[cb], kx);
             }
     };
     const int ngroups = (ntiles + HM_TT - 1) / HM_TT;
@@ -226,7 +279,7 @@
             for (int sub = 0; sub < HM_TT; sub++) {
                 const int tile = grp * HM_TT + sub;
                 if (tile < ntiles) {
-                    hm_v16i acc[HM_CB];
+                    acc_t acc[HM_CB];
                     mma(tile, buf, sub, acc);
                     fold(acc);
                 }
@@ -236,20 +289,38 @@
     }
 #pragma unroll
     for (int cb = 0; cb < HM_CB; cb++) {
-        const int o1 = __shfl_xor(m1[cb], 32, 64), o2 = __shfl_xor(m2[cb], 32, 64);
-        const int b1 = min(m1[cb], o1);
-        const int b2 = min(max(m1[cb], o1), min(m2[cb], o2));
+        const key_t o1 = __shfl_xor(m1[cb], 32, 64), o2 = __shfl_xor(m2[cb], 32, 64);
+        const key_t b1 = min(m1[cb], o1);
+        const key_t b2 = min(max(m1[cb], o1), min(m2[cb], o2));
         const int qi = q0 + 32 * cb + r;
         if (h == 0 && qi < nq) {
             const long long o = (long long)pair * nq + qi;
             const bool live = qi < nqp;
-            const bool has1 = live && b1 < HM_SENT, has2 = live && b2 < HM_SENT;
-            const int bd = has1 ? (b1 >> HM_IDX_BITS) - HM_BIAS + pa[cb] : 256;
-            best_idx[o] = bd < 256 ? (b1 & ((1 << HM_IDX_BITS) - 1)) : -1;
+            const bool has1 = live && b1 < F::sent(), has2 = live && b2 < F::sent();
+            const int k1 = (int)b1, k2 = (int)b2;
+            const int bd = has1 ? (k1 >> HM_IDX_BITS) - HM_BIAS + pa[cb] : 256;
+            best_idx[o] = bd < 256 ? (k1 & ((1 << HM_IDX_BITS) - 1)) : -1;
             best_dist[o] = bd;
-            second_dist[o] = has2 ? (b2 >> HM_IDX_BITS) - HM_BIAS + pa[cb] : 256;
-        }
-    }
+            second_dist[o] = has2 ? (k2 >> HM_IDX_BITS) - HM_BIAS + pa[cb] : 256;
+        }
+    }
+}
+
+__global__ __launch_bounds__(64) void k_fp4_tile(const unsigned* __restrict__ a, const unsigned* __restrict__ b, const float* __restrict__ c,
+                                                 float* __restrict__ out)
+{
+    const int lane = threadIdx.x, h = lane >> 5, r = lane & 31;
+    hm_v16f acc;
+#pragma unroll
+    for (int i = 0; i < 16; i++) acc[i] = c[(i & 3) + 8 * (i >> 2) + 4 * h];
+#pragma unroll
+    for (int s = 0; s < 4; s++) acc = hm_mfma(hm_expand32_fp4(a[8 * r + 4 * h + s], 2u), hm_expand32_fp4(b[8 * r + 4 * h + s], 10u), acc);
+#pragma unroll
+    for (int i = 0; i < 16; i++) out[32 * ((i & 3) + 8 * (i >> 2) + 4 * h) + r] = acc[i];
+}
+void match_launch_fp4_tile(hipStream_t s, const unsigned* a, const unsigned* b, const float* c, float* out)
+{
+    hipLaunchKernelGGL(k_fp4_tile, dim3(1), dim3(64), 0, s, a, b, c, out);
 }
 
 __global__ __launch_bounds__(256) void k_hamming_merge(const unsigned* __restrict__ part_best, const int* __restrict__ part_second,
@@ -751,10 +822,14 @@
                      int nq, int nt, int n_pairs, const int* nq_n, const int* nt_n, int n_split, int variant,
                      unsigned* part_best, int* part_second, int* bi, int* bd, int* sd)
 {
-    if (variant == 3 && nt <= HM_MAX_NT) {
+    if (variant >= 3 && variant <= 5 && nt <= HM_MAX_NT) {
         const int q_blocks = (nq + HM_QW * HM_WAVES - 1) / (HM_QW * HM_WAVES);
-        hipLaunchKernelGGL(k_hamming_mfma, dim3(n_pairs * q_blocks), dim3(HM_TPB), 0, s, q, q_pair_bytes, t, t_pair_bytes, nq, nt, nq_n, nt_n,
-                           q_blocks, bi, bd, sd);
+        if (variant == 4)
+            hipLaunchKernelGGL(k_hamming_mfma<false>, dim3(n_pairs * q_blocks), dim3(HM_TPB), 0, s, q, q_pair_bytes, t, t_pair_bytes, nq, nt, nq_n, nt_n,
+                               q_blocks, bi, bd, sd);
+        else
+            hipLaunchKernelGGL(k_hamming_mfma<true>, dim3(n_pairs * q_blocks), dim3(HM_TPB), 0, s, q, q_pair_bytes, t, t_pair_bytes, nq, nt, nq_n, nt_n,
+                               q_blocks, bi, bd, sd);
         return;
     }
     const dim3 grid(n_pairs * n_split);
diff --git a/motioncheck_ccm_slam_amd/csrc/orb_host.cpp b/motioncheck_ccm_slam_amd/csrc/orb_host.cpp
--- a/motioncheck_ccm_slam_amd/csrc/orb_host.cpp
+++ b/motioncheck_ccm_slam_amd/csrc/orb_host.cpp
@@ -6,11 +6,11 @@
 
 extern "C" hipError_t orb_upload_pattern();
 size_t orb_octree_lds_bytes(int list_cap);
-void orb_launch_resize(hipStream_t, const OrbGeom&, int level, int dw, int dh, int nframes);
+void orb_launch_resize(hipStream_t, const OrbGeom&, int level, int dw, int dh, int nframes, int* clear_status);
 void orb_launch_score(hipStream_t, const OrbGeom&, int ntiles, int nframes);
 void orb_launch_nms(hipStream_t, const OrbGeom&, const OrbCell*, int ncells, int nframes, unsigned* slots, int* cell_count);
 void orb_launch_fast_cells(hipStream_t, const OrbGeom&, const OrbCell*, const OrbBand*, int nbands, int nframes, size_t lds_bytes,
-                           int surv_cap, unsigned* slots, int* cell_count);
+                           int surv_cap, unsigned* slots, int* cell_count, int* clear_status);
 size_t orb_fast_cells_lds(int pitch, int bh, int surv_cap);
 void orb_launch_octree(hipStream_t, const OrbGeom&, const OrbCell*, int nlevels, int nframes, int list_cap,
                        const unsigned* slots, const int* cell_count, unsigned* keysA, unsigned* keysB,
@@ -306,12 +306,17 @@
     const OrbGeom& gd = G;
     const OrbCell* cd = S.cells_dev.as<OrbCell>();
     hipStream_t st = c->stream;
-    if (frame0 == 0) CCM_HIP(c, hipMemsetAsync(S.status.p, 0, 4, st));
-    for (int l = 1; l < G.nlevels; l++) { ProfScope ps(c, CCM_PROF_RESIZE); orb_launch_resize(st, gd, l, G.lv[l].w, G.lv[l].h, nrun); }
+    int* clear = frame0 == 0 ? S.status.as<int>() : nullptr;
+    for (int l = 1; l < G.nlevels; l++) {
+        ProfScope ps(c, CCM_PROF_RESIZE);
+        orb_launch_resize(st, gd, l, G.lv[l].w, G.lv[l].h, nrun, clear);
+        clear = nullptr;
+    }
     if (S.fused && !S.bands.empty()) {
         ProfScope ps(c, CCM_PROF_FAST_SCORE);
-        orb_launch_fast_cells(st, gd, cd, S.bands_dev.as<OrbBand>(), (int)S.bands.size(), nrun, S.band_lds, S.surv_cap, S.slots.as<unsigned>(), S.cell_count.as<int>());
+        orb_launch_fast_cells(st, gd, cd, S.bands_dev.as<OrbBand>(), (int)S.bands.size(), nrun, S.band_lds, S.surv_cap, S.slots.as<unsigned>(), S.cell_count.as<int>(), clear);
     } else {
+        if (clear) CCM_HIP(c, hipMemsetAsync(clear, 0, 4, st));
         { ProfScope ps(c, CCM_PROF_FAST_SCORE); orb_launch_score(st, gd, G.ntiles, nrun); }
         if (G.ncells > 0) { ProfScope ps(c, CCM_PROF_CELL_NMS); orb_launch_nms(st, gd, cd, G.ncells, nrun, S.slots.as<unsigned>(), S.cell_count.as<int>()); }
     }
diff --git a/motioncheck_ccm_slam_amd/csrc/orb_kernels.hip b/motioncheck_ccm_slam_amd/csrc/orb_kernels.hip
--- a/motioncheck_ccm_slam_amd/csrc/orb_kernels.hip
+++ b/motioncheck_ccm_slam_amd/csrc/orb_kernels.hip
@@ -72,8 +72,9 @@
 #ifndef RS_ROWS
 #define RS_ROWS 8
 #endif
-__global__ __launch_bounds__(256) void k_pyr_resize(const OrbGeom g, int level)
-{
+__global__ __launch_bounds__(256) void k_pyr_resize(const OrbGeom g, int level, int* __restrict__ clear_status)
+{
+    if (clear_status && (blockIdx.x | blockIdx.y | blockIdx.z | threadIdx.x) == 0) *clear_status = 0;
     const OrbLevel& D = g.lv[level];
     const OrbLevel& S = g.lv[level - 1];
     const int lane = threadIdx.x & 63;
@@ -411,9 +412,10 @@
 __device__ __forceinline__ int sel4(int ci, const T (&a)[4]) { return ci == 0 ? (int)a[0] : ci == 1 ? (int)a[1] : ci == 2 ? (int)a[2] : (int)a[3]; }
 template <bool PACKED>
 __global__ __launch_bounds__(FC_TPB) __attribute__((amdgpu_waves_per_eu(8, 8))) void k_fast_cells(const OrbGeom g, const OrbCell* __restrict__ cells, const OrbBand* __restrict__ bands,
-                                                    unsigned* __restrict__ slots, int* __restrict__ cell_count, int unused_, int abl, int xcd_on)
+                                                    unsigned* __restrict__ slots, int* __restrict__ cell_count, int* __restrict__ clear_status, int abl, int xcd_on)
 {
     extern __shared__ __attribute__((aligned(16))) uint8_t fc_smem[];
+    if (clear_status && (blockIdx.x | blockIdx.y | threadIdx.x) == 0) *clear_status = 0;
     int wx, wy;
     xcd_work_item(xcd_on, wx, wy);
     FC_STAMP(0);
@@ -1271,10 +1273,10 @@
 
 size_t orb_octree_lds_bytes(int list_cap) { return (size_t)list_cap * OCT_NODE_LDS + 64 + 4 * (size_t)OCT_LDS_KEYS + 8 * (size_t)list_cap; }
 
-void orb_launch_resize(hipStream_t s, const OrbGeom& g_dev, int level, int dw, int dh, int nframes)
+void orb_launch_resize(hipStream_t s, const OrbGeom& g_dev, int level, int dw, int dh, int nframes, int* clear_status)
 {
     dim3 grid((dw + 255) / 256, (dh + 4 * RS_ROWS - 1) / (4 * RS_ROWS), nframes);
-    hipLaunchKernelGGL(k_pyr_resize, grid, dim3(256), 0, s, g_dev, level);
+    hipLaunchKernelGGL(k_pyr_resize, grid, dim3(256), 0, s, g_dev, level, clear_status);
 }
 void orb_launch_score(hipStream_t s, const OrbGeom& g_dev, int ntiles, int nframes)
 {
@@ -1286,7 +1288,7 @@
     hipLaunchKernelGGL(k_cell_nms, dim3((ncells + 3) / 4, nframes), dim3(256), 0, s, g_dev, cells, slots, cell_count);
 }
 void orb_launch_fast_cells(hipStream_t s, const OrbGeom& g_dev, const OrbCell* cells, const OrbBand* bands, int nbands, int nframes,
-                           size_t lds_bytes, int surv_cap, unsigned* slots, int* cell_count)
+                           size_t lds_bytes, int surv_cap, unsigned* slots, int* cell_count, int* clear_status)
 {
     static const bool packed = !(getenv("CCM_FC_PACKED") && atoi(getenv("CCM_FC_PACKED")) == 0);
     static const int abl = getenv("CCM_FC_ABL") ? atoi(getenv("CCM_FC_ABL")) : 0;
@@ -1294,8 +1296,8 @@
     static const size_t lds_min = getenv("CCM_FC_LDS_MIN") ? (size_t)atol(getenv("CCM_FC_LDS_MIN")) : 0;
     if (lds_bytes < lds_min) lds_bytes = lds_min;
     (void)surv_cap;
-    if (packed) hipLaunchKernelGGL(k_fast_cells<true>, dim3(nbands, nframes), dim3(FC_TPB), lds_bytes, s, g_dev, cells, bands, slots, cell_count, 0, abl, xcd_on);
-    else hipLaunchKernelGGL(k_fast_cells<false>, dim3(nbands, nframes), dim3(FC_TPB), lds_bytes, s, g_dev, cells, bands, slots, cell_count, 0, abl, xcd_on);
+    if (packed) hipLaunchKernelGGL(k_fast_cells<true>, dim3(nbands, nframes), dim3(FC_TPB), lds_bytes, s, g_dev, cells, bands, slots, cell_count, clear_status, abl, xcd_on);
+    else hipLaunchKernelGGL(k_fast_cells<false>, dim3(nbands, nframes), dim3(FC_TPB), lds_bytes, s, g_dev, cells, bands, slots, cell_count, clear_status, abl, xcd_on);
 }
 size_t orb_fast_cells_lds(int pitch, int bh, int surv_cap) { return fc_lds_bytes(pitch, bh, surv_cap); }
 void orb_launch_octree(hipStream_t s, const OrbGeom& g_dev, const OrbCell* cells, int nlevels, int nframes, int list_cap,
```

Measured after the change: 293.1 Mfeatures/s, median of 6. 4.0% higher.
